# KKKSQJ/DeepLearning

Hardware: AMD Instinct MI355X
Metric: images/sec (higher is better)
Workload: dtype bf16; 1 GPU; model=resnet50, global_batch=256, image_size=224, parallelism=dp1

## Files before the change

csrc/batchnorm.hip:

```cpp
#include "common.h"
#include "vec.h"

namespace dla {


template <typename dev_t>
__global__ void bn_stats_kernel(const dev_t* __restrict__ x, float* __restrict__ sums,
                                int N, int C, int64_t HW) {
  __shared__ float smem[16];
  const int c = blockIdx.x;
  const int64_t total = (int64_t)N * HW;
  float sum = 0.f, sumsq = 0.f;
  for (int64_t m = (int64_t)blockIdx.y * blockDim.x + threadIdx.x; m < total;
       m += (int64_t)gridDim.y * blockDim.x) {
    const int64_t n = m / HW, hw = m % HW;
    const float f = to_f32(x[(n * C + c) * HW + hw]);
    sum += f;
    sumsq += f * f;
  }
  sum = block_reduce_sum(sum, smem);
  sumsq = block_reduce_sum(sumsq, smem);
  if (threadIdx.x == 0) {
    atomicAdd(&sums[c], sum);
    atomicAdd(&sums[C + c], sumsq);
  }
}

__device__ __forceinline__ void bn_finalize_channel(
    int c, float sum, float sumsq, const float* __restrict__ weight,
    const float* __restrict__ bias, float* __restrict__ mean,
    float* __restrict__ rstd, float* __restrict__ running_mean,
    float* __restrict__ running_var, float* __restrict__ scale,
    float* __restrict__ shift, float count, float eps, float momentum) {
  const float mu = sum / count;
  const float var = fmaxf(sumsq / count - mu * mu, 0.f);
  const float rs = rsqrtf(var + eps);
  mean[c] = mu;
  rstd[c] = rs;
  if (running_mean != nullptr && momentum > 0.f) {
    const float unbiased = var * count / fmaxf(count - 1.f, 1.f);
    running_mean[c] = (1.f - momentum) * running_mean[c] + momentum * mu;
    running_var[c] = (1.f - momentum) * running_var[c] + momentum * unbiased;
  }
  const float sc = weight[c] * rs;
  scale[c] = sc;
  shift[c] = bias[c] - mu * sc;
}

__global__ void bn_finalize_kernel(const float* __restrict__ sums,
                                   const float* __restrict__ weight,
                                   const float* __restrict__ bias,
                                   float* __restrict__ mean, float* __restrict__ rstd,
                                   float* __restrict__ running_mean,
                                   float* __restrict__ running_var,
                                   float* __restrict__ scale, float* __restrict__ shift,
                                   int C, float count, float eps, float momentum) {
  const int c = blockIdx.x * blockDim.x + threadIdx.x;
  if (c >= C) return;
  bn_finalize_channel(c, sums[c], sums[C + c], weight, bias, mean, rstd,
                      running_mean, running_var, scale, shift, count, eps,
                      momentum);
}

constexpr int kFinCh = 16, kFinRows = 64;

__global__ void __launch_bounds__(kFinCh * kFinRows)
bn_finalize_parts_kernel(const float* __restrict__ parts, int n_parts,
                         const float* __restrict__ weight,
                         const float* __restrict__ bias,
                         float* __restrict__ mean, float* __restrict__ rstd,
                         float* __restrict__ running_mean,
                         float* __restrict__ running_var,
                         float* __restrict__ scale, float* __restrict__ shift,
                         int C, float count, float eps, float momentum) {
  __shared__ float ls[2][kFinRows][kFinCh + 1];
  const int cl = threadIdx.x % kFinCh, rl = threadIdx.x / kFinCh;
  const int c = blockIdx.x * kFinCh + cl;
  float s = 0.f, q = 0.f;
  if (c < C) {
#pragma unroll 4
    for (int r = rl; r < n_parts; r += kFinRows) {
      const float* p = parts + (int64_t)r * 2 * C;
      s += p[c];
      q += p[C + c];
    }
  }
  ls[0][rl][cl] = s;
  ls[1][rl][cl] = q;
  __syncthreads();
  for (int h = kFinRows / 2; h > 0; h >>= 1) {
    if (rl < h) {
      ls[0][rl][cl] += ls[0][rl + h][cl];
      ls[1][rl][cl] += ls[1][rl + h][cl];
    }
    __syncthreads();
  }
  if (rl == 0 && c < C)
    bn_finalize_channel(c, ls[0][0][cl], ls[1][0][cl], weight, bias, mean,
                        rstd, running_mean, running_var, scale, shift, count,
                        eps, momentum);
}

template <typename dev_t, int V, bool RELU>
__global__ void bn_apply_kernel(const dev_t* __restrict__ x,
                                const float* __restrict__ scale,
                                const float* __restrict__ shift,
                                dev_t* __restrict__ y, int C, int64_t HW,
                                int64_t n_total) {
  const int64_t stride = (int64_t)gridDim.x * blockDim.x * V;
  for (int64_t i = ((int64_t)blockIdx.x * blockDim.x + threadIdx.x) * V;
       i < n_total; i += stride) {
    const int c = (int)((i / HW) % C);
    const float sc = scale[c], sh = shift[c];
    Vec<dev_t, V> xv = vload<dev_t, V>(x + i);
    Vec<dev_t, V> yv;
#pragma unroll
    for (int j = 0; j < V; ++j) {
      const float f = bn_pre(to_f32(xv.v[j]), sc, sh);
      yv.v[j] = from_f32<dev_t>(RELU ? fmaxf(f, 0.f) : f);
    }
    vstore<dev_t, V>(y + i, yv);
  }
}

template <typename dev_t, bool RELU>
__global__ void bn_bwd_stats_kernel(const dev_t* __restrict__ dy,
                                    const dev_t* __restrict__ x,
                                    const dev_t* __restrict__ y,
                                    const float* __restrict__ mean,
                                    const float* __restrict__ rstd,
                                    float* __restrict__ sums,
                                    int N, int C, int64_t HW) {
  __shared__ float smem[16];
  const int c = blockIdx.x;
  const float mu = mean[c], rs = rstd[c];
  const int64_t total = (int64_t)N * HW;
  float s_dy = 0.f, s_dyxh = 0.f;
  for (int64_t m = (int64_t)blockIdx.y * blockDim.x + threadIdx.x; m < total;
       m += (int64_t)gridDim.y * blockDim.x) {
    const int64_t n = m / HW, hw = m % HW;
    const int64_t idx = (n * C + c) * HW + hw;
    float g = to_f32(dy[idx]);
    if (RELU && to_f32(y[idx]) <= 0.f) g = 0.f;
    const float xh = (to_f32(x[idx]) - mu) * rs;
    s_dy += g;
    s_dyxh += g * xh;
  }
  s_dy = block_reduce_sum(s_dy, smem);
  s_dyxh = block_reduce_sum(s_dyxh, smem);
  if (threadIdx.x == 0) {
    atomicAdd(&sums[c], s_dy);
    atomicAdd(&sums[C + c], s_dyxh);
  }
}

template <typename dev_t, bool RELU>
__global__ void bn_bwd_dx_kernel(const dev_t* __restrict__ dy,
                                 const dev_t* __restrict__ x,
                                 const dev_t* __restrict__ y,
                                 const float* __restrict__ mean,
                                 const float* __restrict__ rstd,
                                 const float* __restrict__ weight,
                                 const float* __restrict__ sums,
                                 dev_t* __restrict__ dx, int C, int64_t HW,
                                 int64_t n_total, float inv_count) {
  const int64_t stride = (int64_t)gridDim.x * blockDim.x;
  for (int64_t i = (int64_t)blockIdx.x * blockDim.x + threadIdx.x; i < n_total;
       i += stride) {
    const int c = (int)((i / HW) % C);
    const float mu = mean[c], rs = rstd[c];
    float g = to_f32(dy[i]);
    if (RELU && to_f32(y[i]) <= 0.f) g = 0.f;
    const float xh = (to_f32(x[i]) - mu) * rs;
    const float m_dy = sums[c] * inv_count;
    const float m_dyxh = sums[C + c] * inv_count;
    dx[i] = from_f32<dev_t>(weight[c] * rs * (g - m_dy - xh * m_dyxh));
  }
}



inline int64_t nhwc_used_threads(int lanes_per_row, int64_t rows,
                                 int64_t target_lanes) {
  int64_t k = target_lanes / lanes_per_row;
  if (k > rows) k = rows;
  if (k < 1) k = 1;
  return (int64_t)lanes_per_row * k;
}

constexpr int kRedThreads = 256;
constexpr int kRedLanes = 32;
constexpr int kRedBlocks = 2048;
constexpr int kRedMaxParts = 512;
constexpr int kRedMinRows = 8;
constexpr int red_unroll(int tensors) { return tensors <= 2 ? 4 : 2; }

#define DLA_RED_KERNEL \
  __launch_bounds__(dla::kRedThreads) __attribute__((amdgpu_waves_per_eu(1, 4)))

struct NhwcRedTile {
  int bl, rb, chunks, parts;
};

inline NhwcRedTile nhwc_red_tile(int lanes_per_row, int64_t rows,
                                 int blocks = kRedBlocks,
                                 int max_parts = kRedMaxParts) {
  NhwcRedTile t;
  t.chunks = (lanes_per_row + kRedLanes - 1) / kRedLanes;
  t.bl = (lanes_per_row + t.chunks - 1) / t.chunks;
  t.rb = kRedThreads / t.bl;
  const int64_t per_part = (int64_t)t.rb * kRedMinRows;
  const int64_t by_rows = (rows + per_part - 1) / per_part;
  const int64_t p = std::min<int64_t>(
      std::min<int64_t>(blocks / t.chunks, max_parts), by_rows);
  t.parts = (int)std::max<int64_t>(p, 1);
  return t;
}

struct NhwcRedPos {
  int c0;
  int64_t row;
  int64_t rstride;
  bool active;
};

template <int V>
__device__ __forceinline__ NhwcRedPos nhwc_red_pos(int C, int bl, int rb) {
  const int lane = threadIdx.x % bl, rl = threadIdx.x / bl;
  const int gl = blockIdx.x * bl + lane;
  NhwcRedPos p;
  p.c0 = gl * V;
  p.row = (int64_t)blockIdx.y * rb + rl;
  p.rstride = (int64_t)gridDim.y * rb;
  p.active = rl < rb && gl < C / V;
  return p;
}

template <int U, typename L, typename A>
__device__ __forceinline__ void nhwc_red_rows(const NhwcRedPos& p,
                                              int64_t rows, L&& load, A&& add) {
  if (!p.active) return;
  using D = decltype(load(int64_t{}));
  int64_t r = p.row;
  for (; r + (U - 1) * p.rstride < rows; r += U * p.rstride) {
    D d[U];
#pragma unroll
    for (int u = 0; u < U; ++u) d[u] = load(r + u * p.rstride);
#pragma unroll
    for (int u = 0; u < U; ++u) add(r + u * p.rstride, d[u]);
  }
  for (; r < rows; r += p.rstride) add(r, load(r));
}

template <int V, int NS>
__device__ __forceinline__ void nhwc_red_tail(const float (&acc)[NS][V],
                                              float* __restrict__ slab, int C,
                                              int bl, int rb) {
  __shared__ __attribute__((aligned(16))) float ls[kRedThreads * V];
  const int W = bl * V;
  const int cbase = blockIdx.x * W;
  float* out = slab + (int64_t)blockIdx.y * NS * C;
#pragma unroll
  for (int s = 0; s < NS; ++s) {
    if (s) __syncthreads();
    if ((int)threadIdx.x < bl * rb) {
#pragma unroll
      for (int j = 0; j < V; ++j) ls[threadIdx.x * V + j] = acc[s][j];
    }
    __syncthreads();
    for (int col = threadIdx.x; col < W; col += kRedThreads) {
      if (cbase + col < C) {
        float sum = 0.f;
        for (int r = 0; r < rb; ++r) sum += ls[r * W + col];
        out[s * C + cbase + col] = sum;
      }
    }
  }
}

constexpr int kSlabCols = 32, kSlabRows = 32;

__global__ void __launch_bounds__(kSlabCols * kSlabRows)
bn_slab_reduce_kernel(const float* __restrict__ slab, int n_parts, int n_cols,
                      float* __restrict__ sums) {
  __shared__ float ls[kSlabRows][kSlabCols + 1];
  const int cl = threadIdx.x % kSlabCols, rl = threadIdx.x / kSlabCols;
  const int c = blockIdx.x * kSlabCols + cl;
  float s = 0.f;
  if (c < n_cols) {
#pragma unroll 4
    for (int r = rl; r < n_parts; r += kSlabRows)
      s += slab[(int64_t)r * n_cols + c];
  }
  ls[rl][cl] = s;
  __syncthreads();
  for (int h = kSlabRows / 2; h > 0; h >>= 1) {
    if (rl < h) ls[rl][cl] += ls[rl + h][cl];
    __syncthreads();
  }
  if (rl == 0 && c < n_cols) sums[c] = ls[0][cl];
}

constexpr int kSlabGroup = 128;
constexpr int kSlabDeep = kRedMaxParts;

__global__ void __launch_bounds__(kSlabCols * kSlabRows)
bn_slab_group_reduce_kernel(const float* __restrict__ slab, int n_parts,
                            int n_cols, float* __restrict__ groups) {
  __shared__ float ls[kSlabRows][kSlabCols + 1];
  const int cl = threadIdx.x % kSlabCols, rl = threadIdx.x / kSlabCols;
  const int c = blockIdx.x * kSlabCols + cl;
  const int r0 = blockIdx.y * kSlabGroup;
  const int r1 = r0 + kSlabGroup < n_parts ? r0 + kSlabGroup : n_parts;
  float s = 0.f;
  if (c < n_cols) {
#pragma unroll 4
    for (int r = r0 + rl; r < r1; r += kSlabRows)
      s += slab[(int64_t)r * n_cols + c];
  }
  ls[rl][cl] = s;
  __syncthreads();
  for (int h = kSlabRows / 2; h > 0; h >>= 1) {
    if (rl < h) ls[rl][cl] += ls[rl + h][cl];
    __syncthreads();
  }
  if (rl == 0 && c < n_cols) groups[(int64_t)blockIdx.y * n_cols + c] = ls[0][cl];
}

template <typename dev_t, int V>
__global__ void DLA_RED_KERNEL
bn_stats_nhwc_kernel(const dev_t* __restrict__ x, float* __restrict__ slab,
                     int C, int64_t rows, int bl, int rb) {
  const NhwcRedPos p = nhwc_red_pos<V>(C, bl, rb);
  float acc[2][V];
#pragma unroll
  for (int j = 0; j < V; ++j) { acc[0][j] = 0.f; acc[1][j] = 0.f; }
  nhwc_red_rows<red_unroll(1)>(
      p, rows, [&](int64_t r) { return vload<dev_t, V>(x + r * C + p.c0); },
      [&](int64_t, const Vec<dev_t, V>& xv) {
#pragma unroll
        for (int j = 0; j < V; ++j) {
          const float f = to_f32(xv.v[j]);
          acc[0][j] += f;
          acc[1][j] += f * f;
        }
      });
  nhwc_red_tail<V, 2>(acc, slab, C, bl, rb);
}

template <typename dev_t, int V, bool RELU>
__global__ void bn_apply_nhwc_kernel(const dev_t* __restrict__ x,
                                     const float* __restrict__ scale,
                                     const float* __restrict__ shift,
                                     dev_t* __restrict__ y, int C, int64_t rows,
                                     int64_t used) {
  const int64_t t = (int64_t)blockIdx.x * blockDim.x + threadIdx.x;
  if (t >= used) return;
  const int lanes_per_row = C / V;
  const int c0 = (int)(t % lanes_per_row) * V;
  const int64_t rstride = used / lanes_per_row;
  float sc[V], sh[V];
#pragma unroll
  for (int j = 0; j < V; ++j) { sc[j] = scale[c0 + j]; sh[j] = shift[c0 + j]; }
  for (int64_t r = t / lanes_per_row; r < rows; r += rstride) {
    Vec<dev_t, V> xv = vload<dev_t, V>(x + r * C + c0);
    Vec<dev_t, V> yv;
#pragma unroll
    for (int j = 0; j < V; ++j) {
      const float f = bn_pre(to_f32(xv.v[j]), sc[j], sh[j]);
      yv.v[j] = from_f32<dev_t>(RELU ? fmaxf(f, 0.f) : f);
    }
    vstore<dev_t, V>(y + r * C + c0, yv);
  }
}

template <typename dev_t, int V, bool RELU, bool MASK_Y = false>
__global__ void DLA_RED_KERNEL
bn_bwd_stats_nhwc_kernel(const dev_t* __restrict__ dy,
                         const dev_t* __restrict__ x,
                         const dev_t* __restrict__ y,
                         const float* __restrict__ scale,
                         const float* __restrict__ shift,
                         const float* __restrict__ mean,
                         const float* __restrict__ rstd,
                         float* __restrict__ slab, int C, int64_t rows, int bl,
                         int rb) {
  const NhwcRedPos p = nhwc_red_pos<V>(C, bl, rb);
  float mu[V], rs[V], sc[V], sh[V];
  float acc[2][V];
#pragma unroll
  for (int j = 0; j < V; ++j) {
    mu[j] = p.active ? mean[p.c0 + j] : 0.f;
    rs[j] = p.active ? rstd[p.c0 + j] : 0.f;
    sc[j] = (p.active && RELU && !MASK_Y) ? scale[p.c0 + j] : 0.f;
    sh[j] = (p.active && RELU && !MASK_Y) ? shift[p.c0 + j] : 0.f;
    acc[0][j] = 0.f;
    acc[1][j] = 0.f;
  }
  struct Row {
    Vec<dev_t, V> dy, x, y;
  };
  nhwc_red_rows<red_unroll(MASK_Y ? 3 : 2)>(
      p, rows,
      [&](int64_t r) {
        const int64_t base = r * C + p.c0;
        Row d;
        d.dy = vload<dev_t, V>(dy + base);
        d.x = vload<dev_t, V>(x + base);
        if (RELU && MASK_Y) d.y = vload<dev_t, V>(y + base);
        return d;
      },
      [&](int64_t, const Row& d) {
#pragma unroll
        for (int j = 0; j < V; ++j) {
          float g = to_f32(d.dy.v[j]);
          const float xf = to_f32(d.x.v[j]);
          if (RELU && MASK_Y && to_f32(d.y.v[j]) <= 0.f) g = 0.f;
          if (RELU && !MASK_Y && !(bn_pre(xf, sc[j], sh[j]) > 0.f)) g = 0.f;
          const float xh = (xf - mu[j]) * rs[j];
          acc[0][j] += g;
          acc[1][j] += g * xh;
        }
      });
  nhwc_red_tail<V, 2>(acc, slab, C, bl, rb);
}

template <typename dev_t, int V, bool RELU, bool MASK_Y = false>
__global__ void bn_bwd_dx_nhwc_kernel(const dev_t* __restrict__ dy,
                                      const dev_t* __restrict__ x,
                                      const dev_t* __restrict__ y,
                                      const float* __restrict__ scale,
                                      const float* __restrict__ shift,
                                      const float* __restrict__ mean,
                                      const float* __restrict__ rstd,
                                      const float* __restrict__ weight,
                                      const float* __restrict__ sums,
                                      dev_t* __restrict__ dx, int C,
                                      int64_t rows, int64_t used,
                                      float inv_count) {
  const int64_t t = (int64_t)blockIdx.x * blockDim.x + threadIdx.x;
  if (t >= used) return;
  const int lanes_per_row = C / V;
  const int c0 = (int)(t % lanes_per_row) * V;
  const int64_t rstride = used / lanes_per_row;
  float mu[V], rs[V], wr[V], sc[V], sh[V], m_dy[V], m_dyxh[V];
#pragma unroll
  for (int j = 0; j < V; ++j) {
    mu[j] = mean[c0 + j];
    rs[j] = rstd[c0 + j];
    wr[j] = weight[c0 + j] * rs[j];
    sc[j] = (RELU && !MASK_Y) ? scale[c0 + j] : 0.f;
    sh[j] = (RELU && !MASK_Y) ? shift[c0 + j] : 0.f;
    m_dy[j] = sums[c0 + j] * inv_count;
    m_dyxh[j] = sums[C + c0 + j] * inv_count;
  }
  for (int64_t r = t / lanes_per_row; r < rows; r += rstride) {
    const int64_t base = r * C + c0;
    Vec<dev_t, V> dyv = vload<dev_t, V>(dy + base);
    Vec<dev_t, V> xv = vload<dev_t, V>(x + base);
    Vec<dev_t, V> yv;
    if (RELU && MASK_Y) yv = vload<dev_t, V>(y + base);
    Vec<dev_t, V> dxv;
#pragma unroll
    for (int j = 0; j < V; ++j) {
      float g = to_f32(dyv.v[j]);
      const float xf = to_f32(xv.v[j]);
      if (RELU && MASK_Y && to_f32(yv.v[j]) <= 0.f) g = 0.f;
      if (RELU && !MASK_Y && !(bn_pre(xf, sc[j], sh[j]) > 0.f)) g = 0.f;
      const float xh = (xf - mu[j]) * rs[j];
      dxv.v[j] = from_f32<dev_t>(wr[j] * (g - m_dy[j] - xh * m_dyxh[j]));
    }
    vstore<dev_t, V>(dx + r * C + c0, dxv);
  }
}

template <typename dev_t, int V, bool DUAL>
__global__ void bn_add_relu_nhwc_kernel(const dev_t* __restrict__ x,
                                        const float* __restrict__ scale,
                                        const float* __restrict__ shift,
                                        const dev_t* __restrict__ idn,
                                        const float* __restrict__ scale_d,
                                        const float* __restrict__ shift_d,
                                        dev_t* __restrict__ out, int C,
                                        int64_t rows, int64_t used) {
  const int64_t t = (int64_t)blockIdx.x * blockDim.x + threadIdx.x;
  if (t >= used) return;
  const int lanes_per_row = C / V;
  const int c0 = (int)(t % lanes_per_row) * V;
  const int64_t rstride = used / lanes_per_row;
  float sc[V], sh[V], scd[V];
#pragma unroll
  for (int j = 0; j < V; ++j) {
    sc[j] = scale[c0 + j];
    sh[j] = shift[c0 + j];
    if (DUAL) {
      scd[j] = scale_d[c0 + j];
      sh[j] += shift_d[c0 + j];
    }
  }
  for (int64_t r = t / lanes_per_row; r < rows; r += rstride) {
    const int64_t base = r * C + c0;
    Vec<dev_t, V> xv = vload<dev_t, V>(x + base);
    Vec<dev_t, V> iv = vload<dev_t, V>(idn + base);
    Vec<dev_t, V> ov;
#pragma unroll
    for (int j = 0; j < V; ++j) {
      float f = to_f32(xv.v[j]) * sc[j] + sh[j];
      f += DUAL ? to_f32(iv.v[j]) * scd[j] : to_f32(iv.v[j]);
      ov.v[j] = from_f32<dev_t>(fmaxf(f, 0.f));
    }
    vstore<dev_t, V>(out + base, ov);
  }
}

template <typename dev_t, int V, bool DUAL>
__global__ void DLA_RED_KERNEL
bn_join_bwd_stats_nhwc_kernel(
    const dev_t* __restrict__ dy, const dev_t* __restrict__ out,
    const dev_t* __restrict__ x, const float* __restrict__ mean,
    const float* __restrict__ rstd, const dev_t* __restrict__ xd,
    const float* __restrict__ mean_d, const float* __restrict__ rstd_d,
    dev_t* __restrict__ g_out, float* __restrict__ slab, int C, int64_t rows,
    int bl, int rb) {
  constexpr int NS = DUAL ? 3 : 2;
  const NhwcRedPos p = nhwc_red_pos<V>(C, bl, rb);
  float mu[V], rs[V], mud[V], rsd[V];
  float acc[NS][V];
#pragma unroll
  for (int j = 0; j < V; ++j) {
    mu[j] = p.active ? mean[p.c0 + j] : 0.f;
    rs[j] = p.active ? rstd[p.c0 + j] : 0.f;
    mud[j] = (p.active && DUAL) ? mean_d[p.c0 + j] : 0.f;
    rsd[j] = (p.active && DUAL) ? rstd_d[p.c0 + j] : 0.f;
#pragma unroll
    for (int s = 0; s < NS; ++s) acc[s][j] = 0.f;
  }
  struct Row {
    Vec<dev_t, V> dy, out, x, xd;
  };
  nhwc_red_rows<red_unroll(DUAL ? 4 : 3)>(
      p, rows,
      [&](int64_t r) {
        const int64_t base = r * C + p.c0;
        Row d;
        d.dy = vload<dev_t, V>(dy + base);
        d.out = vload<dev_t, V>(out + base);
        d.x = vload<dev_t, V>(x + base);
        if (DUAL) d.xd = vload<dev_t, V>(xd + base);
        return d;
      },
      [&](int64_t r, const Row& d) {
        Vec<dev_t, V> gv;
#pragma unroll
        for (int j = 0; j < V; ++j) {
          const bool on = to_f32(d.out.v[j]) > 0.f;
          gv.v[j] = on ? d.dy.v[j] : from_f32<dev_t>(0.f);
          const float g = on ? to_f32(d.dy.v[j]) : 0.f;
          acc[0][j] += g;
          acc[1][j] += g * ((to_f32(d.x.v[j]) - mu[j]) * rs[j]);
          if (DUAL)
            acc[NS - 1][j] += g * ((to_f32(d.xd.v[j]) - mud[j]) * rsd[j]);
        }
        vstore<dev_t, V>(g_out + r * C + p.c0, gv);
      });
  nhwc_red_tail<V, NS>(acc, slab, C, bl, rb);
}

template <typename dev_t, int V>
__global__ void bn_join_bwd_dx_dual_nhwc_kernel(
    const dev_t* __restrict__ g, const dev_t* __restrict__ x,
    const dev_t* __restrict__ xd, const float* __restrict__ mean,
    const float* __restrict__ rstd, const float* __restrict__ weight,
    const float* __restrict__ mean_d, const float* __restrict__ rstd_d,
    const float* __restrict__ weight_d, const float* __restrict__ sums,
    dev_t* __restrict__ dx, dev_t* __restrict__ dxd, int C, int64_t rows,
    int64_t used, float inv_count) {
  const int64_t t = (int64_t)blockIdx.x * blockDim.x + threadIdx.x;
  if (t >= used) return;
  const int lanes_per_row = C / V;
  const int c0 = (int)(t % lanes_per_row) * V;
  const int64_t rstride = used / lanes_per_row;
  float mu[V], rs[V], wr[V], mud[V], rsd[V], wrd[V], m_g[V], m_gxh[V],
      m_gxhd[V];
#pragma unroll
  for (int j = 0; j < V; ++j) {
    mu[j] = mean[c0 + j];
    rs[j] = rstd[c0 + j];
    wr[j] = weight[c0 + j] * rs[j];
    mud[j] = mean_d[c0 + j];
    rsd[j] = rstd_d[c0 + j];
    wrd[j] = weight_d[c0 + j] * rsd[j];
    m_g[j] = sums[c0 + j] * inv_count;
    m_gxh[j] = sums[C + c0 + j] * inv_count;
    m_gxhd[j] = sums[2 * C + c0 + j] * inv_count;
  }
  for (int64_t r = t / lanes_per_row; r < rows; r += rstride) {
    const int64_t base = r * C + c0;
    Vec<dev_t, V> gv = vload<dev_t, V>(g + base);
    Vec<dev_t, V> xv = vload<dev_t, V>(x + base);
    Vec<dev_t, V> xdv = vload<dev_t, V>(xd + base);
    Vec<dev_t, V> dxv, dxdv;
#pragma unroll
    for (int j = 0; j < V; ++j) {
      const float gg = to_f32(gv.v[j]) - m_g[j];
      const float xh = (to_f32(xv.v[j]) - mu[j]) * rs[j];
      const float xhd = (to_f32(xdv.v[j]) - mud[j]) * rsd[j];
      dxv.v[j] = from_f32<dev_t>(wr[j] * (gg - xh * m_gxh[j]));
      dxdv.v[j] = from_f32<dev_t>(wrd[j] * (gg - xhd * m_gxhd[j]));
    }
    vstore<dev_t, V>(dx + base, dxv);
    vstore<dev_t, V>(dxd + base, dxdv);
  }
}

inline bool is_nhwc(const torch::Tensor& t) {
  return t.dim() == 4 && t.is_contiguous(at::MemoryFormat::ChannelsLast) &&
         !t.is_contiguous();
}

struct BnFinalized {
  torch::Tensor mean, rstd, scale, shift;
};

inline BnFinalized bn_finalize_launch(
    const torch::Tensor& sums, const torch::Tensor& weight,
    const torch::Tensor& bias, c10::optional<torch::Tensor>& running_mean,
    c10::optional<torch::Tensor>& running_var, int C, int64_t rows,
    double momentum, double eps) {
  TORCH_CHECK(sums.is_cuda() && sums.scalar_type() == torch::kFloat &&
                  sums.is_contiguous(),
              "bn sums must be a contiguous fp32 GPU tensor");
  TORCH_CHECK((sums.dim() == 1 && sums.size(0) == 2 * C) ||
                  (sums.dim() == 2 && sums.size(0) >= 1 &&
                   sums.size(1) == 2 * C),
              "bn sums must be [2C] or [n_parts, 2C]");
  TORCH_CHECK(weight.numel() == C && bias.numel() == C,
              "bn weight/bias must have C elements");
  auto opts_f = sums.options();
  BnFinalized f{torch::empty({C}, opts_f), torch::empty({C}, opts_f),
                torch::empty({C}, opts_f), torch::empty({C}, opts_f)};
  auto w32 = weight.to(torch::kFloat).contiguous();
  auto b32 = bias.to(torch::kFloat).contiguous();
  float* rm = running_mean.has_value() ? running_mean->data_ptr<float>() : nullptr;
  float* rv = running_var.has_value() ? running_var->data_ptr<float>() : nullptr;
  const int n_parts = sums.dim() == 2 ? (int)sums.size(0) : 1;
  if (n_parts > 1) {
    hipLaunchKernelGGL(bn_finalize_parts_kernel, dim3((C + kFinCh - 1) / kFinCh),
                       dim3(kFinCh * kFinRows), 0, stream(),
                       sums.data_ptr<float>(), n_parts, w32.data_ptr<float>(),
                       b32.data_ptr<float>(), f.mean.data_ptr<float>(),
                       f.rstd.data_ptr<float>(), rm, rv,
                       f.scale.data_ptr<float>(), f.shift.data_ptr<float>(), C,
                       (float)rows, (float)eps, (float)momentum);
  } else {
    hipLaunchKernelGGL(bn_finalize_kernel, dim3((C + 255) / 256), dim3(256), 0,
                       stream(), sums.data_ptr<float>(), w32.data_ptr<float>(),
                       b32.data_ptr<float>(), f.mean.data_ptr<float>(),
                       f.rstd.data_ptr<float>(), rm, rv,
                       f.scale.data_ptr<float>(), f.shift.data_ptr<float>(), C,
                       (float)rows, (float)eps, (float)momentum);
  }
  return f;
}

inline torch::Tensor bn_param_grad(const torch::Tensor& sums, int64_t offset,
                                   int C, const torch::Tensor& weight) {
  return sums.narrow(0, offset, C).to(weight.scalar_type());
}

inline torch::Tensor bn_slab_reduce_launch(const torch::Tensor& slab) {
  const int n_parts = (int)slab.size(0), n_cols = (int)slab.size(1);
  if (n_parts > kSlabDeep) {
    const int groups = (n_parts + kSlabGroup - 1) / kSlabGroup;
    auto part = torch::empty({groups, n_cols}, slab.options());
    hipLaunchKernelGGL(bn_slab_group_reduce_kernel,
                       dim3((n_cols + kSlabCols - 1) / kSlabCols, groups),
                       dim3(kSlabCols * kSlabRows), 0, stream(),
                       slab.data_ptr<float>(), n_parts, n_cols,
                       part.data_ptr<float>());
    return bn_slab_reduce_launch(part);
  }
  auto sums = torch::empty({n_cols}, slab.options());
  hipLaunchKernelGGL(bn_slab_reduce_kernel,
                     dim3((n_cols + kSlabCols - 1) / kSlabCols),
                     dim3(kSlabCols * kSlabRows), 0, stream(),
                     slab.data_ptr<float>(), n_parts, n_cols,
                     sums.data_ptr<float>());
  return sums;
}

inline bool is_nhwc_rows(const torch::Tensor& t) {
  return t.dim() == 4 && t.is_contiguous(at::MemoryFormat::ChannelsLast);
}

}

std::vector<torch::Tensor> batchnorm_fwd(torch::Tensor x, torch::Tensor weight,
                                         torch::Tensor bias,
                                         c10::optional<torch::Tensor> running_mean,
                                         c10::optional<torch::Tensor> running_var,
                                         double momentum, double eps, bool relu) {
  DLA_CHECK_CUDA(x);
  TORCH_CHECK(x.dim() == 4, "batchnorm_fwd expects a 4D tensor");
  const bool nhwc = dla::is_nhwc(x);
  TORCH_CHECK(nhwc || x.is_contiguous(), "batchnorm_fwd: x must be contiguous "
              "(NCHW or channels_last)");
  const int N = (int)x.size(0), C = (int)x.size(1);
  const int64_t HW = x.size(2) * x.size(3);
  auto opts_f = x.options().dtype(torch::kFloat);
  auto sums = nhwc ? torch::Tensor() : torch::zeros({2 * C}, opts_f);
  auto mean = torch::empty({C}, opts_f);
  auto rstd = torch::empty({C}, opts_f);
  auto scale = torch::empty({C}, opts_f);
  auto shift = torch::empty({C}, opts_f);
  auto y = torch::empty_like(x);
  auto w32 = weight.to(torch::kFloat);
  auto b32 = bias.to(torch::kFloat);

  const int64_t rows = (int64_t)N * HW;
  const int ysplit = (int)std::min<int64_t>((rows + 65535) / 65536 + 1,
                                            std::max(1, 2048 / C));
  DLA_DISPATCH_FLOAT_TYPES(x.scalar_type(), "batchnorm_fwd", [&] {
    if (nhwc) {
      constexpr int VM = 16 / (int)sizeof(dev_t);
      auto stats = [&](auto vtag) {
        constexpr int V = decltype(vtag)::value;
        const auto t = dla::nhwc_red_tile(C / V, rows);
        sums = torch::empty({t.parts, 2 * C}, opts_f);
        hipLaunchKernelGGL((dla::bn_stats_nhwc_kernel<dev_t, V>),
                           dim3(t.chunks, t.parts), dim3(dla::kRedThreads), 0,
                           dla::stream(), (const dev_t*)x.data_ptr(),
                           sums.data_ptr<float>(), C, rows, t.bl, t.rb);
      };
      if (C % VM == 0) stats(std::integral_constant<int, VM>{});
      else if (C % 2 == 0) stats(std::integral_constant<int, 2>{});
      else stats(std::integral_constant<int, 1>{});
    } else {
      hipLaunchKernelGGL((dla::bn_stats_kernel<dev_t>), dim3(C, ysplit), dim3(256), 0,
                         dla::stream(), (const dev_t*)x.data_ptr(),
                         sums.data_ptr<float>(), N, C, HW);
    }
    float* rm = running_mean.has_value() ? running_mean->data_ptr<float>() : nullptr;
    float* rv = running_var.has_value() ? running_var->data_ptr<float>() : nullptr;
    if (sums.dim() == 2 && sums.size(0) > 1) {
      hipLaunchKernelGGL(dla::bn_finalize_parts_kernel,
                         dim3((C + dla::kFinCh - 1) / dla::kFinCh),
                         dim3(dla::kFinCh * dla::kFinRows), 0, dla::stream(),
                         sums.data_ptr<float>(), (int)sums.size(0),
                         w32.data_ptr<float>(), b32.data_ptr<float>(),
                         mean.data_ptr<float>(), rstd.data_ptr<float>(), rm, rv,
                         scale.data_ptr<float>(), shift.data_ptr<float>(), C,
                         (float)rows, (float)eps, (float)momentum);
    } else {
      hipLaunchKernelGGL(dla::bn_finalize_kernel, dim3((C + 255) / 256), dim3(256), 0,
                         dla::stream(), sums.data_ptr<float>(), w32.data_ptr<float>(),
                         b32.data_ptr<float>(), mean.data_ptr<float>(),
                         rstd.data_ptr<float>(), rm, rv,
                         scale.data_ptr<float>(), shift.data_ptr<float>(), C,
                         (float)rows, (float)eps, (float)momentum);
    }
    const int64_t n_total = x.numel();
    constexpr int VMAX = 16 / (int)sizeof(dev_t);
    auto launch = [&](auto vtag, auto rtag) {
      constexpr int V = decltype(vtag)::value;
      constexpr bool R = decltype(rtag)::value;
      if (nhwc) {
        const int lanes = C / V;
        const int64_t used = dla::nhwc_used_threads(lanes, rows, 524288);
        hipLaunchKernelGGL((dla::bn_apply_nhwc_kernel<dev_t, V, R>),
                           dim3((int)((used + 255) / 256)), dim3(256), 0,
                           dla::stream(), (const dev_t*)x.data_ptr(),
                           scale.data_ptr<float>(), shift.data_ptr<float>(),
                           (dev_t*)y.data_ptr(), C, rows, used);
        return;
      }
      const int grid = dla::grid_1d((n_total + V - 1) / V, 256);
      if (false) ;
      else
        hipLaunchKernelGGL((dla::bn_apply_kernel<dev_t, V, R>), dim3(grid), dim3(256),
                           0, dla::stream(), (const dev_t*)x.data_ptr(),
                           scale.data_ptr<float>(), shift.data_ptr<float>(),
                           (dev_t*)y.data_ptr(), C, HW, n_total);
    };
    const bool vec_ok = nhwc ? (C % VMAX == 0) : (HW % VMAX == 0);
    if (vec_ok) {
      if (relu) launch(std::integral_constant<int, VMAX>{}, std::true_type{});
      else launch(std::integral_constant<int, VMAX>{}, std::false_type{});
    } else {
      if (relu) launch(std::integral_constant<int, 1>{}, std::true_type{});
      else launch(std::integral_constant<int, 1>{}, std::false_type{});
    }
  });
  HIP_CHECK_ERR();
  return {y, mean, rstd, scale, shift};
}

std::vector<torch::Tensor> batchnorm_fwd_from_sums(
    torch::Tensor x, torch::Tensor weight, torch::Tensor bias,
    torch::Tensor sums, c10::optional<torch::Tensor> running_mean,
    c10::optional<torch::Tensor> running_var, double momentum, double eps,
    bool relu) {
  DLA_CHECK_CUDA(x);
  TORCH_CHECK(x.dim() == 4, "batchnorm_fwd_from_sums expects a 4D tensor");
  const bool nhwc = dla::is_nhwc(x);
  TORCH_CHECK(nhwc || x.is_contiguous(),
              "batchnorm_fwd_from_sums: x must be contiguous");
  const int N = (int)x.size(0), C = (int)x.size(1);
  const int64_t HW = x.size(2) * x.size(3);
  auto y = torch::empty_like(x);
  const int64_t rows = (int64_t)N * HW;
  auto fin = dla::bn_finalize_launch(sums, weight, bias, running_mean,
                                     running_var, C, rows, momentum, eps);
  auto& mean = fin.mean;
  auto& rstd = fin.rstd;
  auto& scale = fin.scale;
  auto& shift = fin.shift;
  DLA_DISPATCH_FLOAT_TYPES(x.scalar_type(), "batchnorm_fwd_from_sums", [&] {
    const int64_t n_total = x.numel();
    constexpr int VMAX = 16 / (int)sizeof(dev_t);
    auto launch = [&](auto vtag, auto rtag) {
      constexpr int V = decltype(vtag)::value;
      constexpr bool R = decltype(rtag)::value;
      if (nhwc) {
        const int lanes = C / V;
        const int64_t used = dla::nhwc_used_threads(lanes, rows, 524288);
        hipLaunchKernelGGL((dla::bn_apply_nhwc_kernel<dev_t, V, R>),
                           dim3((int)((used + 255) / 256)), dim3(256), 0,
                           dla::stream(), (const dev_t*)x.data_ptr(),
                           scale.data_ptr<float>(), shift.data_ptr<float>(),
                           (dev_t*)y.data_ptr(), C, rows, used);
        return;
      }
      const int grid = dla::grid_1d((n_total + V - 1) / V, 256);
      hipLaunchKernelGGL((dla::bn_apply_kernel<dev_t, V, R>), dim3(grid),
                         dim3(256), 0, dla::stream(),
                         (const dev_t*)x.data_ptr(), scale.data_ptr<float>(),
                         shift.data_ptr<float>(), (dev_t*)y.data_ptr(), C, HW,
                         n_total);
    };
    const bool vec_ok = nhwc ? (C % VMAX == 0) : (HW % VMAX == 0);
    if (vec_ok) {
      if (relu) launch(std::integral_constant<int, VMAX>{}, std::true_type{});
      else launch(std::integral_constant<int, VMAX>{}, std::false_type{});
    } else {
      if (relu) launch(std::integral_constant<int, 1>{}, std::true_type{});
      else launch(std::integral_constant<int, 1>{}, std::false_type{});
    }
  });
  HIP_CHECK_ERR();
  return {y, mean, rstd, scale, shift};
}

torch::Tensor bn_apply(torch::Tensor x, torch::Tensor scale, torch::Tensor shift,
                       bool relu) {
  DLA_CHECK_CUDA(x);
  TORCH_CHECK(x.dim() == 4, "bn_apply expects a 4D tensor");
  const bool nhwc = dla::is_nhwc(x);
  TORCH_CHECK(nhwc || x.is_contiguous(), "bn_apply: x must be contiguous");
  const int C = (int)x.size(1);
  const int64_t HW = x.size(2) * x.size(3);
  auto y = torch::empty_like(x);
  auto sc = scale.to(torch::kFloat).contiguous();
  auto sh = shift.to(torch::kFloat).contiguous();
  const int64_t n_total = x.numel();
  DLA_DISPATCH_FLOAT_TYPES(x.scalar_type(), "bn_apply", [&] {
    constexpr int VMAX = 16 / (int)sizeof(dev_t);
    auto launch = [&](auto vtag, auto rtag) {
      constexpr int V = decltype(vtag)::value;
      constexpr bool R = decltype(rtag)::value;
      if (nhwc) {
        const int64_t rows = n_total / C;
        const int lanes = C / V;
        const int64_t used = dla::nhwc_used_threads(lanes, rows, 524288);
        hipLaunchKernelGGL((dla::bn_apply_nhwc_kernel<dev_t, V, R>),
                           dim3((int)((used + 255) / 256)), dim3(256), 0,
                           dla::stream(), (const dev_t*)x.data_ptr(),
                           sc.data_ptr<float>(), sh.data_ptr<float>(),
                           (dev_t*)y.data_ptr(), C, rows, used);
        return;
      }
      const int grid = dla::grid_1d((n_total + V - 1) / V, 256);
      if (false) ;
      else
        hipLaunchKernelGGL((dla::bn_apply_kernel<dev_t, V, R>), dim3(grid), dim3(256),
                           0, dla::stream(), (const dev_t*)x.data_ptr(),
                           sc.data_ptr<float>(), sh.data_ptr<float>(),
                           (dev_t*)y.data_ptr(), C, HW, n_total);
    };
    const bool vec_ok = nhwc ? (C % VMAX == 0) : (HW % VMAX == 0);
    if (vec_ok) {
      if (relu) launch(std::integral_constant<int, VMAX>{}, std::true_type{});
      else launch(std::integral_constant<int, VMAX>{}, std::false_type{});
    } else {
      if (relu) launch(std::integral_constant<int, 1>{}, std::true_type{});
      else launch(std::integral_constant<int, 1>{}, std::false_type{});
    }
  });
  HIP_CHECK_ERR();
  return y;
}

bool bn_relu_mask_from_x(torch::Tensor x) { return dla::is_nhwc(x); }

std::vector<torch::Tensor> batchnorm_bwd_ex(
    torch::Tensor dy, torch::Tensor x, c10::optional<torch::Tensor> y,
    torch::Tensor weight, torch::Tensor mean, torch::Tensor rstd,
    c10::optional<torch::Tensor> scale, c10::optional<torch::Tensor> shift,
    bool relu) {
  DLA_CHECK_CUDA(dy); DLA_CHECK_CUDA(x);
  const bool nhwc = dla::is_nhwc(x);
  TORCH_CHECK(nhwc || x.is_contiguous(), "batchnorm_bwd: x must be contiguous");
  if (nhwc && !dla::is_nhwc(dy)) dy = dy.contiguous(at::MemoryFormat::ChannelsLast);
  if (!nhwc) dy = dy.contiguous();
  const int N = (int)x.size(0), C = (int)x.size(1);
  const int64_t HW = x.size(2) * x.size(3);
  const int64_t rows = (int64_t)N * HW;
  auto opts_f = x.options().dtype(torch::kFloat);
  auto sums = nhwc ? torch::Tensor() : torch::zeros({2 * C}, opts_f);
  auto dx = torch::empty_like(x);
  auto w32 = weight.to(torch::kFloat);
  const int ysplit = (int)std::min<int64_t>((rows + 65535) / 65536 + 1,
                                            std::max(1, 2048 / C));
  const bool mask_y = relu && y.has_value();
  if (relu && !mask_y) {
    TORCH_CHECK(bn_relu_mask_from_x(x) && scale.has_value() && shift.has_value(),
                "batchnorm_bwd: the relu mask needs y, or channels_last x "
                "with the forward's scale and shift");
    for (const auto* t : {&*scale, &*shift})
      TORCH_CHECK(t->is_cuda() && t->scalar_type() == torch::kFloat &&
                      t->is_contiguous() && t->numel() == C,
                  "batchnorm_bwd: scale/shift must be contiguous fp32 [C]");
  }
  if (mask_y)
    TORCH_CHECK(y->scalar_type() == x.scalar_type() && y->sizes() == x.sizes() &&
                    (nhwc ? dla::is_nhwc(*y) : y->is_contiguous()),
                "batchnorm_bwd: y must match x (shape, dtype, layout)");
  const float* scp = (relu && !mask_y) ? scale->data_ptr<float>() : nullptr;
  const float* shp = (relu && !mask_y) ? shift->data_ptr<float>() : nullptr;
  DLA_DISPATCH_FLOAT_TYPES(x.scalar_type(), "batchnorm_bwd", [&] {
    const dev_t* yp = mask_y ? (const dev_t*)y->data_ptr() : nullptr;
    auto with_mode = [&](auto f) {
      if (!relu) f(std::false_type{}, std::false_type{});
      else if (mask_y) f(std::true_type{}, std::true_type{});
      else f(std::true_type{}, std::false_type{});
    };
    with_mode([&](auto rtag, auto mtag) {
      constexpr bool R = decltype(rtag)::value;
      constexpr bool MY = decltype(mtag)::value;
      if (nhwc) {
        constexpr int VM = 16 / (int)sizeof(dev_t);
        auto stats = [&](auto vtag) {
          constexpr int V = decltype(vtag)::value;
          const auto t = dla::nhwc_red_tile(C / V, rows);
          auto slab = torch::empty({t.parts, 2 * C}, opts_f);
          hipLaunchKernelGGL((dla::bn_bwd_stats_nhwc_kernel<dev_t, V, R, MY>),
                             dim3(t.chunks, t.parts), dim3(dla::kRedThreads),
                             0, dla::stream(), (const dev_t*)dy.data_ptr(),
                             (const dev_t*)x.data_ptr(), yp, scp, shp,
                             mean.data_ptr<float>(), rstd.data_ptr<float>(),
                             slab.data_ptr<float>(), C, rows, t.bl, t.rb);
          sums = dla::bn_slab_reduce_launch(slab);
        };
        if (C % VM == 0) stats(std::integral_constant<int, VM>{});
        else if (C % 2 == 0) stats(std::integral_constant<int, 2>{});
        else stats(std::integral_constant<int, 1>{});
      } else if constexpr (!R || MY) {
        hipLaunchKernelGGL((dla::bn_bwd_stats_kernel<dev_t, R>), dim3(C, ysplit),
                           dim3(256), 0, dla::stream(), (const dev_t*)dy.data_ptr(),
                           (const dev_t*)x.data_ptr(), yp, mean.data_ptr<float>(),
                           rstd.data_ptr<float>(), sums.data_ptr<float>(), N, C, HW);
      }
    });

    const int64_t n_total = x.numel();
    const float inv_count = 1.f / (float)rows;
    constexpr int VMAX = 16 / (int)sizeof(dev_t);
    with_mode([&](auto rtag, auto mtag) {
      constexpr bool R = decltype(rtag)::value;
      constexpr bool MY = decltype(mtag)::value;
      if (nhwc) {
        auto dxk = [&](auto vtag) {
          constexpr int V = decltype(vtag)::value;
          const int lanes = C / V;
          const int64_t used = dla::nhwc_used_threads(lanes, rows, 524288);
          hipLaunchKernelGGL((dla::bn_bwd_dx_nhwc_kernel<dev_t, V, R, MY>),
                             dim3((int)((used + 255) / 256)), dim3(256), 0,
                             dla::stream(), (const dev_t*)dy.data_ptr(),
                             (const dev_t*)x.data_ptr(), yp, scp, shp,
                             mean.data_ptr<float>(), rstd.data_ptr<float>(),
                             w32.data_ptr<float>(), sums.data_ptr<float>(),
                             (dev_t*)dx.data_ptr(), C, rows, used, inv_count);
        };
        if (C % VMAX == 0) dxk(std::integral_constant<int, VMAX>{});
        else dxk(std::integral_constant<int, 1>{});
      } else if constexpr (!R || MY) {
        hipLaunchKernelGGL((dla::bn_bwd_dx_kernel<dev_t, R>), dim3(dla::grid_1d(n_total, 256)),
                           dim3(256), 0, dla::stream(), (const dev_t*)dy.data_ptr(),
                           (const dev_t*)x.data_ptr(), yp, mean.data_ptr<float>(),
                           rstd.data_ptr<float>(), w32.data_ptr<float>(),
                           sums.data_ptr<float>(), (dev_t*)dx.data_ptr(), C, HW,
                           n_total, inv_count);
      }
    });
  });
  HIP_CHECK_ERR();
  return {dx, dla::bn_param_grad(sums, C, C, weight),
          dla::bn_param_grad(sums, 0, C, weight)};
}

std::vector<torch::Tensor> batchnorm_bwd(torch::Tensor dy, torch::Tensor x,
                                         c10::optional<torch::Tensor> y,
                                         torch::Tensor weight, torch::Tensor mean,
                                         torch::Tensor rstd, bool relu) {
  TORCH_CHECK(!relu || y.has_value(), "batchnorm_bwd: relu mask needs y");
  return batchnorm_bwd_ex(dy, x, relu ? y : c10::nullopt, weight, mean, rstd,
                          c10::nullopt, c10::nullopt, relu);
}

namespace dla {

inline void join_check(const torch::Tensor& x, const torch::Tensor& other,
                       const char* what) {
  TORCH_CHECK(other.is_cuda() && other.scalar_type() == x.scalar_type() &&
                  other.sizes() == x.sizes() && is_nhwc_rows(other),
              "bn join: ", what, " must match x (shape, dtype, channels_last)");
}

inline int join_vec(const torch::Tensor& x) {
  const int vmax = 16 / (int)x.element_size();
  TORCH_CHECK(x.size(1) % vmax == 0,
              "bn join: C must be a multiple of ", vmax);
  return vmax;
}

}

std::vector<torch::Tensor> bn_add_relu_fwd_from_sums(
    torch::Tensor x, torch::Tensor weight, torch::Tensor bias,
    torch::Tensor sums, c10::optional<torch::Tensor> running_mean,
    c10::optional<torch::Tensor> running_var, double momentum, double eps,
    torch::Tensor identity) {
  DLA_CHECK_CUDA(x);
  TORCH_CHECK(dla::is_nhwc_rows(x), "bn_add_relu: x must be channels_last");
  dla::join_check(x, identity, "identity");
  dla::join_vec(x);
  const int C = (int)x.size(1);
  const int64_t rows = x.numel() / C;
  auto fin = dla::bn_finalize_launch(sums, weight, bias, running_mean,
                                     running_var, C, rows, momentum, eps);
  auto out = torch::empty_like(x);
  DLA_DISPATCH_FLOAT_TYPES(x.scalar_type(), "bn_add_relu_fwd_from_sums", [&] {
    constexpr int V = 16 / (int)sizeof(dev_t);
    const int64_t used = dla::nhwc_used_threads(C / V, rows, 524288);
    hipLaunchKernelGGL((dla::bn_add_relu_nhwc_kernel<dev_t, V, false>),
                       dim3((int)((used + 255) / 256)), dim3(256), 0,
                       dla::stream(), (const dev_t*)x.data_ptr(),
                       fin.scale.data_ptr<float>(), fin.shift.data_ptr<float>(),
                       (const dev_t*)identity.data_ptr(), nullptr, nullptr,
                       (dev_t*)out.data_ptr(), C, rows, used);
  });
  HIP_CHECK_ERR();
  return {out, fin.mean, fin.rstd};
}

std::vector<torch::Tensor> bn_add_relu_dual_fwd_from_sums(
    torch::Tensor x, torch::Tensor weight, torch::Tensor bias,
    torch::Tensor sums, c10::optional<torch::Tensor> running_mean,
    c10::optional<torch::Tensor> running_var, double momentum, double eps,
    torch::Tensor xd, torch::Tensor weight_d, torch::Tensor bias_d,
    torch::Tensor sums_d, c10::optional<torch::Tensor> running_mean_d,
    c10::optional<torch::Tensor> running_var_d, double momentum_d,
    double eps_d) {
  DLA_CHECK_CUDA(x);
  TORCH_CHECK(dla::is_nhwc_rows(x), "bn_add_relu_dual: x must be channels_last");
  dla::join_check(x, xd, "xd");
  dla::join_vec(x);
  const int C = (int)x.size(1);
  const int64_t rows = x.numel() / C;
  auto fin = dla::bn_finalize_launch(sums, weight, bias, running_mean,
                                     running_var, C, rows, momentum, eps);
  auto fd = dla::bn_finalize_launch(sums_d, weight_d, bias_d, running_mean_d,
                                    running_var_d, C, rows, momentum_d, eps_d);
  auto out = torch::empty_like(x);
  DLA_DISPATCH_FLOAT_TYPES(x.scalar_type(), "bn_add_relu_dual_fwd_from_sums", [&] {
    constexpr int V = 16 / (int)sizeof(dev_t);
    const int64_t used = dla::nhwc_used_threads(C / V, rows, 524288);
    hipLaunchKernelGGL((dla::bn_add_relu_nhwc_kernel<dev_t, V, true>),
                       dim3((int)((used + 255) / 256)), dim3(256), 0,
                       dla::stream(), (const dev_t*)x.data_ptr(),
                       fin.scale.data_ptr<float>(), fin.shift.data_ptr<float>(),
                       (const dev_t*)xd.data_ptr(), fd.scale.data_ptr<float>(),
                       fd.shift.data_ptr<float>(), (dev_t*)out.data_ptr(), C,
                       rows, used);
  });
  HIP_CHECK_ERR();
  return {out, fin.mean, fin.rstd, fd.mean, fd.rstd};
}

std::vector<torch::Tensor> bn_add_relu_bwd(torch::Tensor dy, torch::Tensor out,
                                           torch::Tensor x, torch::Tensor weight,
                                           torch::Tensor mean,
                                           torch::Tensor rstd) {
  DLA_CHECK_CUDA(x);
  TORCH_CHECK(dla::is_nhwc_rows(x), "bn_add_relu_bwd: x must be channels_last");
  dla::join_check(x, out, "out");
  if (!dla::is_nhwc_rows(dy)) dy = dy.contiguous(at::MemoryFormat::ChannelsLast);
  dla::join_check(x, dy, "dy");
  dla::join_vec(x);
  const int C = (int)x.size(1);
  const int64_t rows = x.numel() / C;
  TORCH_CHECK(mean.numel() == C && rstd.numel() == C && weight.numel() == C,
              "bn_add_relu_bwd: per-channel tensors must have C elements");
  torch::Tensor sums;
  auto g = torch::empty_like(x);
  auto dx = torch::empty_like(x);
  auto w32 = weight.to(torch::kFloat).contiguous();
  DLA_DISPATCH_FLOAT_TYPES(x.scalar_type(), "bn_add_relu_bwd", [&] {
    constexpr int V = 16 / (int)sizeof(dev_t);
    const int lanes = C / V;
    const auto t = dla::nhwc_red_tile(lanes, rows);
    auto slab = torch::empty({t.parts, 2 * C},
                             x.options().dtype(torch::kFloat));
    hipLaunchKernelGGL((dla::bn_join_bwd_stats_nhwc_kernel<dev_t, V, false>),
                       dim3(t.chunks, t.parts), dim3(dla::kRedThreads), 0,
                       dla::stream(),
                       (const dev_t*)dy.data_ptr(), (const dev_t*)out.data_ptr(),
                       (const dev_t*)x.data_ptr(), mean.data_ptr<float>(),
                       rstd.data_ptr<float>(), nullptr, nullptr, nullptr,
                       (dev_t*)g.data_ptr(), slab.data_ptr<float>(), C, rows,
                       t.bl, t.rb);
    sums = dla::bn_slab_reduce_launch(slab);
    const int64_t used = dla::nhwc_used_threads(lanes, rows, 524288);
    hipLaunchKernelGGL((dla::bn_bwd_dx_nhwc_kernel<dev_t, V, false>),
                       dim3((int)((used + 255) / 256)), dim3(256), 0,
                       dla::stream(), (const dev_t*)g.data_ptr(),
                       (const dev_t*)x.data_ptr(), nullptr, nullptr, nullptr,
                       mean.data_ptr<float>(), rstd.data_ptr<float>(),
                       w32.data_ptr<float>(), sums.data_ptr<float>(),
                       (dev_t*)dx.data_ptr(), C, rows, used,
                       1.f / (float)rows);
  });
  HIP_CHECK_ERR();
  return {g, dx, dla::bn_param_grad(sums, C, C, weight),
          dla::bn_param_grad(sums, 0, C, weight)};
}

std::vector<torch::Tensor> bn_add_relu_dual_bwd(
    torch::Tensor dy, torch::Tensor out, torch::Tensor x, torch::Tensor weight,
    torch::Tensor mean, torch::Tensor rstd, torch::Tensor xd,
    torch::Tensor weight_d, torch::Tensor mean_d, torch::Tensor rstd_d) {
  DLA_CHECK_CUDA(x);
  TORCH_CHECK(dla::is_nhwc_rows(x), "bn_add_relu_dual_bwd: x must be channels_last");
  dla::join_check(x, out, "out");
  dla::join_check(x, xd, "xd");
  if (!dla::is_nhwc_rows(dy)) dy = dy.contiguous(at::MemoryFormat::ChannelsLast);
  dla::join_check(x, dy, "dy");
  dla::join_vec(x);
  const int C = (int)x.size(1);
  const int64_t rows = x.numel() / C;
  TORCH_CHECK(mean.numel() == C && rstd.numel() == C && weight.numel() == C &&
                  mean_d.numel() == C && rstd_d.numel() == C &&
                  weight_d.numel() == C,
              "bn_add_relu_dual_bwd: per-channel tensors must have C elements");
  torch::Tensor sums;
  auto g = torch::empty_like(x);
  auto dx = torch::empty_like(x);
  auto dxd = torch::empty_like(x);
  auto w32 = weight.to(torch::kFloat).contiguous();
  auto wd32 = weight_d.to(torch::kFloat).contiguous();
  DLA_DISPATCH_FLOAT_TYPES(x.scalar_type(), "bn_add_relu_dual_bwd", [&] {
    constexpr int V = 16 / (int)sizeof(dev_t);
    const int lanes = C / V;
    const auto t = dla::nhwc_red_tile(lanes, rows);
    auto slab = torch::empty({t.parts, 3 * C},
                             x.options().dtype(torch::kFloat));
    hipLaunchKernelGGL((dla::bn_join_bwd_stats_nhwc_kernel<dev_t, V, true>),
                       dim3(t.chunks, t.parts), dim3(dla::kRedThreads), 0,
                       dla::stream(),
                       (const dev_t*)dy.data_ptr(), (const dev_t*)out.data_ptr(),
                       (const dev_t*)x.data_ptr(), mean.data_ptr<float>(),
                       rstd.data_ptr<float>(), (const dev_t*)xd.data_ptr(),
                       mean_d.data_ptr<float>(), rstd_d.data_ptr<float>(),
                       (dev_t*)g.data_ptr(), slab.data_ptr<float>(), C, rows,
                       t.bl, t.rb);
    sums = dla::bn_slab_reduce_launch(slab);
    const int64_t used = dla::nhwc_used_threads(lanes, rows, 524288);
    hipLaunchKernelGGL((dla::bn_join_bwd_dx_dual_nhwc_kernel<dev_t, V>),
                       dim3((int)((used + 255) / 256)), dim3(256), 0,
                       dla::stream(), (const dev_t*)g.data_ptr(),
                       (const dev_t*)x.data_ptr(), (const dev_t*)xd.data_ptr(),
                       mean.data_ptr<float>(), rstd.data_ptr<float>(),
                       w32.data_ptr<float>(), mean_d.data_ptr<float>(),
                       rstd_d.data_ptr<float>(), wd32.data_ptr<float>(),
                       sums.data_ptr<float>(), (dev_t*)dx.data_ptr(),
                       (dev_t*)dxd.data_ptr(), C, rows, used,
                       1.f / (float)rows);
  });
  HIP_CHECK_ERR();
  auto dbias = dla::bn_param_grad(sums, 0, C, weight);
  return {dx, dxd, dla::bn_param_grad(sums, C, C, weight), dbias,
          dla::bn_param_grad(sums, 2 * C, C, weight_d),
          dbias.to(weight_d.scalar_type()).clone()};
}

namespace dla {

inline void dx_only_check(const torch::Tensor& x, const torch::Tensor& g,
                          const torch::Tensor& slab, int ns) {
  TORCH_CHECK(is_nhwc_rows(x), "bn dx-only: x must be channels_last");
  join_check(x, g, "g");
  TORCH_CHECK(x.scalar_type() == torch::kBFloat16, "bn dx-only: bf16 only");
  TORCH_CHECK(slab.is_cuda() && slab.scalar_type() == torch::kFloat &&
                  slab.dim() == 2 && slab.is_contiguous() &&
                  slab.size(0) >= 1 && slab.size(1) == ns * x.size(1),
              "bn dx-only: slab must be fp32 [n_parts, ", ns, "*C]");
}

}

torch::Tensor bn_slab_reduce(torch::Tensor slab) {
  TORCH_CHECK(slab.is_cuda() && slab.scalar_type() == torch::kFloat &&
                  slab.dim() == 2 && slab.is_contiguous() && slab.size(0) >= 1,
              "bn_slab_reduce: slab must be a contiguous fp32 [n_parts, n_cols] "
              "GPU tensor");
  auto sums = dla::bn_slab_reduce_launch(slab);
  HIP_CHECK_ERR();
  return sums;
}

std::vector<torch::Tensor> bn_bwd_dx_from_slab(torch::Tensor g,
                                               torch::Tensor slab,
                                               torch::Tensor x,
                                               torch::Tensor weight,
                                               torch::Tensor mean,
                                               torch::Tensor rstd) {
  DLA_CHECK_CUDA(x);
  dla::dx_only_check(x, g, slab, 2);
  const int V = dla::join_vec(x);
  const int C = (int)x.size(1);
  const int64_t rows = x.numel() / C;
  TORCH_CHECK(mean.numel() == C && rstd.numel() == C && weight.numel() == C,
              "bn_bwd_dx_from_slab: per-channel tensors must have C elements");
  auto dx = torch::empty_like(x);
  auto w32 = weight.to(torch::kFloat).contiguous();
  auto sums = dla::bn_slab_reduce_launch(slab);
  using dev_t = __hip_bfloat16;
  const int64_t used = dla::nhwc_used_threads(C / V, rows, 524288);
  hipLaunchKernelGGL((dla::bn_bwd_dx_nhwc_kernel<dev_t, 8, false>),
                     dim3((int)((used + 255) / 256)), dim3(256), 0,
                     dla::stream(), (const dev_t*)g.data_ptr(),
                     (const dev_t*)x.data_ptr(), nullptr, nullptr, nullptr,
                     mean.data_ptr<float>(), rstd.data_ptr<float>(),
                     w32.data_ptr<float>(), sums.data_ptr<float>(),
                     (dev_t*)dx.data_ptr(), C, rows, used, 1.f / (float)rows);
  HIP_CHECK_ERR();
  return {dx, dla::bn_param_grad(sums, C, C, weight),
          dla::bn_param_grad(sums, 0, C, weight)};
}

std::vector<torch::Tensor> bn_join_dual_bwd_dx_from_slab(
    torch::Tensor g, torch::Tensor slab, torch::Tensor x, torch::Tensor weight,
    torch::Tensor mean, torch::Tensor rstd, torch::Tensor xd,
    torch::Tensor weight_d, torch::Tensor mean_d, torch::Tensor rstd_d) {
  DLA_CHECK_CUDA(x);
  dla::dx_only_check(x, g, slab, 3);
  dla::join_check(x, xd, "xd");
  const int V = dla::join_vec(x);
  const int C = (int)x.size(1);
  const int64_t rows = x.numel() / C;
  TORCH_CHECK(mean.numel() == C && rstd.numel() == C && weight.numel() == C &&
                  mean_d.numel() == C && rstd_d.numel() == C &&
                  weight_d.numel() == C,
              "bn_join_dual_bwd_dx_from_slab: per-channel tensors must have C "
              "elements");
  auto dx = torch::empty_like(x);
  auto dxd = torch::empty_like(x);
  auto w32 = weight.to(torch::kFloat).contiguous();
  auto wd32 = weight_d.to(torch::kFloat).contiguous();
  auto sums = dla::bn_slab_reduce_launch(slab);
  using dev_t = __hip_bfloat16;
  const int64_t used = dla::nhwc_used_threads(C / V, rows, 524288);
  hipLaunchKernelGGL((dla::bn_join_bwd_dx_dual_nhwc_kernel<dev_t, 8>),
                     dim3((int)((used + 255) / 256)), dim3(256), 0,
                     dla::stream(), (const dev_t*)g.data_ptr(),
                     (const dev_t*)x.data_ptr(), (const dev_t*)xd.data_ptr(),
                     mean.data_ptr<float>(), rstd.data_ptr<float>(),
                     w32.data_ptr<float>(), mean_d.data_ptr<float>(),
                     rstd_d.data_ptr<float>(), wd32.data_ptr<float>(),
                     sums.data_ptr<float>(), (dev_t*)dx.data_ptr(),
                     (dev_t*)dxd.data_ptr(), C, rows, used,
                     1.f / (float)rows);
  HIP_CHECK_ERR();
  auto dbias = dla::bn_param_grad(sums, 0, C, weight);
  return {dx, dxd, dla::bn_param_grad(sums, C, C, weight), dbias,
          dla::bn_param_grad(sums, 2 * C, C, weight_d),
          dbias.to(weight_d.scalar_type()).clone()};
}

namespace dla {

constexpr int kPoolRun = 8;

template <typename dev_t, int V>
__global__ void __launch_bounds__(256)
bn_relu_maxpool_fwd_nhwc_kernel(const dev_t* __restrict__ x,
                                const float* __restrict__ scale,
                                const float* __restrict__ shift,
                                dev_t* __restrict__ out,
                                uint8_t* __restrict__ slots, int C, int H,
                                int W, int OH, int OW, int runs_per_img) {
  const int n = blockIdx.x / runs_per_img;
  const int oh0 = (blockIdx.x % runs_per_img) * kPoolRun;
  const int oh1 = min(oh0 + kPoolRun, OH);
  const int lanes = C / V;
  const int items = (oh1 - oh0) * OW * lanes;
  const dev_t* xn = x + (int64_t)n * H * W * C;
  const int64_t obase = ((int64_t)n * OH + oh0) * OW * C;
  for (int i = threadIdx.x; i < items; i += blockDim.x) {
    const int c0 = (i % lanes) * V;
    const int p = i / lanes;
    const int ow = p % OW, oh = oh0 + p / OW;
    float sc[V], sh[V], best[V];
    int slot[V];
#pragma unroll
    for (int j = 0; j < V; ++j) {
      sc[j] = scale[c0 + j];
      sh[j] = shift[c0 + j];
      best[j] = -INFINITY;
      slot[j] = 4;
    }
#pragma unroll
    for (int kh = 0; kh < 3; ++kh) {
      const int ih = 2 * oh - 1 + kh;
      if (ih < 0 || ih >= H) continue;
#pragma unroll
      for (int kw = 0; kw < 3; ++kw) {
        const int iw = 2 * ow - 1 + kw;
        if (iw < 0 || iw >= W) continue;
        Vec<dev_t, V> xv =
            vload<dev_t, V>(xn + ((int64_t)ih * W + iw) * C + c0);
#pragma unroll
        for (int j = 0; j < V; ++j) {
          const float f = bn_pre(to_f32(xv.v[j]), sc[j], sh[j]);
          const float y = to_f32(from_f32<dev_t>(fmaxf(f, 0.f)));
          if (y > best[j]) {
            best[j] = y;
            slot[j] = kh * 3 + kw;
          }
        }
      }
    }
    Vec<dev_t, V> ov;
    Vec<uint8_t, V> sv;
#pragma unroll
    for (int j = 0; j < V; ++j) {
      ov.v[j] = from_f32<dev_t>(best[j]);
      sv.v[j] = (uint8_t)slot[j];
    }
    const int64_t o = obase + (int64_t)p * C + c0;
    vstore<dev_t, V>(out + o, ov);
    vstore<uint8_t, V>(slots + o, sv);
  }
}

template <typename dev_t, int V>
__device__ __forceinline__ void stem_pool_grad(
    const dev_t* __restrict__ dpool, const uint8_t* __restrict__ slots,
    const Vec<dev_t, V>& xv, const float* sc, const float* sh, int n, int h,
    int w, int c0, int C, int OH, int OW, float* g) {
#pragma unroll
  for (int j = 0; j < V; ++j) g[j] = 0.f;
  const int oh_hi = min((h + 1) >> 1, OH - 1);
  const int ow_hi = min((w + 1) >> 1, OW - 1);
  for (int oh = h >> 1; oh <= oh_hi; ++oh) {
    const int kh = h - 2 * oh + 1;
    for (int ow = w >> 1; ow <= ow_hi; ++ow) {
      const int want = kh * 3 + (w - 2 * ow + 1);
      const int64_t o = (((int64_t)n * OH + oh) * OW + ow) * C + c0;
      Vec<uint8_t, V> sv = vload<uint8_t, V>(slots + o);
      Vec<dev_t, V> dv = vload<dev_t, V>(dpool + o);
#pragma unroll
      for (int j = 0; j < V; ++j)
        if ((int)sv.v[j] == want) g[j] += to_f32(dv.v[j]);
    }
  }
#pragma unroll
  for (int j = 0; j < V; ++j)
    if (!(bn_pre(to_f32(xv.v[j]), sc[j], sh[j]) > 0.f)) g[j] = 0.f;
}

constexpr int kStemRedBlocks = 1024;

template <typename dev_t, int V>
__global__ void __launch_bounds__(kRedThreads)
bn_relu_maxpool_bwd_stats_nhwc_kernel(
    const dev_t* __restrict__ dpool, const uint8_t* __restrict__ slots,
    const dev_t* __restrict__ x, const float* __restrict__ scale,
    const float* __restrict__ shift, const float* __restrict__ mean,
    const float* __restrict__ rstd, float* __restrict__ slab, int C, int H,
    int W, int OH, int OW, int64_t rows, int bl, int rb) {
  const NhwcRedPos p = nhwc_red_pos<V>(C, bl, rb);
  float mu[V], rs[V], sc[V], sh[V];
  float acc[2][V];
#pragma unroll
  for (int j = 0; j < V; ++j) {
    mu[j] = p.active ? mean[p.c0 + j] : 0.f;
    rs[j] = p.active ? rstd[p.c0 + j] : 0.f;
    sc[j] = p.active ? scale[p.c0 + j] : 0.f;
    sh[j] = p.active ? shift[p.c0 + j] : 0.f;
    acc[0][j] = 0.f;
    acc[1][j] = 0.f;
  }
  nhwc_red_rows<1>(
      p, rows, [&](int64_t r) { return vload<dev_t, V>(x + r * C + p.c0); },
      [&](int64_t r, const Vec<dev_t, V>& xv) {
        const uint32_t r32 = (uint32_t)r;
        const uint32_t q = r32 / (uint32_t)W;
        const int w = (int)(r32 - q * (uint32_t)W);
        const int n = (int)(q / (uint32_t)H);
        const int h = (int)(q - (uint32_t)n * (uint32_t)H);
        float g[V];
        stem_pool_grad<dev_t, V>(dpool, slots, xv, sc, sh, n, h, w, p.c0, C,
                                 OH, OW, g);
#pragma unroll
        for (int j = 0; j < V; ++j) {
          const float xh = (to_f32(xv.v[j]) - mu[j]) * rs[j];
          acc[0][j] += g[j];
          acc[1][j] += g[j] * xh;
        }
      });
  nhwc_red_tail<V, 2>(acc, slab, C, bl, rb);
}

template <typename dev_t, int V>
__global__ void bn_relu_maxpool_bwd_dx_nhwc_kernel(
    const dev_t* __restrict__ dpool, const uint8_t* __restrict__ slots,
    const dev_t* __restrict__ x, const float* __restrict__ scale,
    const float* __restrict__ shift, const float* __restrict__ mean,
    const float* __restrict__ rstd, const float* __restrict__ weight,
    const float* __restrict__ sums, dev_t* __restrict__ dx, int C, int H,
    int W, int OH, int OW, int64_t rows, int64_t used, float inv_count) {
  const int64_t t = (int64_t)blockIdx.x * blockDim.x + threadIdx.x;
  if (t >= used) return;
  const int lanes_per_row = C / V;
  const int c0 = (int)(t % lanes_per_row) * V;
  const int64_t rstride = used / lanes_per_row;
  float mu[V], rs[V], wr[V], sc[V], sh[V], m_g[V], m_gxh[V], g[V];
#pragma unroll
  for (int j = 0; j < V; ++j) {
    mu[j] = mean[c0 + j];
    rs[j] = rstd[c0 + j];
    wr[j] = weight[c0 + j] * rs[j];
    sc[j] = scale[c0 + j];
    sh[j] = shift[c0 + j];
    m_g[j] = sums[c0 + j] * inv_count;
    m_gxh[j] = sums[C + c0 + j] * inv_count;
  }
  for (int64_t r = t / lanes_per_row; r < rows; r += rstride) {
    const uint32_t r32 = (uint32_t)r;
    const uint32_t q = r32 / (uint32_t)W;
    const int w = (int)(r32 - q * (uint32_t)W);
    const int n = (int)(q / (uint32_t)H);
    const int h = (int)(q - (uint32_t)n * (uint32_t)H);
    Vec<dev_t, V> xv = vload<dev_t, V>(x + r * C + c0);
    stem_pool_grad<dev_t, V>(dpool, slots, xv, sc, sh, n, h, w, c0, C, OH, OW,
                             g);
    Vec<dev_t, V> dxv;
#pragma unroll
    for (int j = 0; j < V; ++j) {
      const float xh = (to_f32(xv.v[j]) - mu[j]) * rs[j];
      dxv.v[j] = from_f32<dev_t>(wr[j] * (g[j] - m_g[j] - xh * m_gxh[j]));
    }
    vstore<dev_t, V>(dx + r * C + c0, dxv);
  }
}

inline void stem_check(const torch::Tensor& x, const char* fn) {
  TORCH_CHECK(x.is_cuda() && x.dim() == 4 && is_nhwc_rows(x), fn,
              ": x must be a channels_last 4D GPU tensor");
  const int vmax = 16 / (int)x.element_size();
  TORCH_CHECK(x.size(1) % vmax == 0, fn, ": C must be a multiple of ", vmax);
  TORCH_CHECK(x.numel() > 0 && x.numel() / x.size(1) < (int64_t(1) << 31),
              fn, ": N*H*W must be in [1, 2^31)");
}

}

std::vector<torch::Tensor> bn_relu_maxpool_fwd(
    torch::Tensor x, torch::Tensor weight, torch::Tensor bias,
    c10::optional<torch::Tensor> running_mean,
    c10::optional<torch::Tensor> running_var, double momentum, double eps) {
  dla::stem_check(x, "bn_relu_maxpool_fwd");
  const int N = (int)x.size(0), C = (int)x.size(1);
  const int H = (int)x.size(2), W = (int)x.size(3);
  const int OH = (H - 1) / 2 + 1, OW = (W - 1) / 2 + 1;
  const int64_t rows = (int64_t)N * H * W;
  auto out_opts = x.options().memory_format(at::MemoryFormat::ChannelsLast);
  auto pooled = torch::empty({N, C, OH, OW}, out_opts);
  auto slots = torch::empty({N, C, OH, OW}, out_opts.dtype(torch::kByte));
  const int runs = (OH + dla::kPoolRun - 1) / dla::kPoolRun;
  TORCH_CHECK((int64_t)N * runs < (int64_t(1) << 31),
              "bn_relu_maxpool_fwd: too many blocks");
  dla::BnFinalized fin;
  DLA_DISPATCH_FLOAT_TYPES(x.scalar_type(), "bn_relu_maxpool_fwd", [&] {
    constexpr int V = 16 / (int)sizeof(dev_t);
    const auto t = dla::nhwc_red_tile(C / V, rows);
    auto sums = torch::empty({t.parts, 2 * C},
                             x.options().dtype(torch::kFloat));
    hipLaunchKernelGGL((dla::bn_stats_nhwc_kernel<dev_t, V>),
                       dim3(t.chunks, t.parts), dim3(dla::kRedThreads), 0,
                       dla::stream(), (const dev_t*)x.data_ptr(),
                       sums.data_ptr<float>(), C, rows, t.bl, t.rb);
    fin = dla::bn_finalize_launch(sums, weight, bias, running_mean,
                                  running_var, C, rows, momentum, eps);
    hipLaunchKernelGGL((dla::bn_relu_maxpool_fwd_nhwc_kernel<dev_t, V>),
                       dim3(N * runs), dim3(256), 0, dla::stream(),
                       (const dev_t*)x.data_ptr(), fin.scale.data_ptr<float>(),
                       fin.shift.data_ptr<float>(), (dev_t*)pooled.data_ptr(),
                       slots.data_ptr<uint8_t>(), C, H, W, OH, OW, runs);
  });
  HIP_CHECK_ERR();
  return {pooled, slots, fin.mean, fin.rstd, fin.scale, fin.shift};
}

std::vector<torch::Tensor> bn_relu_maxpool_bwd(
    torch::Tensor dpool, torch::Tensor x, torch::Tensor slots,
    torch::Tensor weight, torch::Tensor mean, torch::Tensor rstd,
    torch::Tensor scale, torch::Tensor shift) {
  dla::stem_check(x, "bn_relu_maxpool_bwd");
  const int N = (int)x.size(0), C = (int)x.size(1);
  const int H = (int)x.size(2), W = (int)x.size(3);
  const int OH = (H - 1) / 2 + 1, OW = (W - 1) / 2 + 1;
  const int64_t rows = (int64_t)N * H * W;
  DLA_CHECK_CUDA(dpool);
  if (!dla::is_nhwc_rows(dpool))
    dpool = dpool.contiguous(at::MemoryFormat::ChannelsLast);
  const std::vector<int64_t> pshape{N, C, OH, OW};
  TORCH_CHECK(dpool.scalar_type() == x.scalar_type() &&
                  dpool.sizes() == at::IntArrayRef(pshape),
              "bn_relu_maxpool_bwd: dpool must be [N, C, OH, OW] of x's dtype");
  TORCH_CHECK(slots.is_cuda() && slots.scalar_type() == torch::kByte &&
                  slots.sizes() == at::IntArrayRef(pshape) &&
                  dla::is_nhwc_rows(slots),
              "bn_relu_maxpool_bwd: slots must be channels_last uint8 "
              "[N, C, OH, OW]");
  for (const auto* t : {&mean, &rstd, &scale, &shift})
    TORCH_CHECK(t->is_cuda() && t->scalar_type() == torch::kFloat &&
                    t->is_contiguous() && t->numel() == C,
                "bn_relu_maxpool_bwd: per-channel tensors must be contiguous "
                "fp32 [C]");
  TORCH_CHECK(weight.numel() == C, "bn_relu_maxpool_bwd: weight must be [C]");
  torch::Tensor sums;
  auto dx = torch::empty_like(x);
  auto w32 = weight.to(torch::kFloat).contiguous();
  DLA_DISPATCH_FLOAT_TYPES(x.scalar_type(), "bn_relu_maxpool_bwd", [&] {
    constexpr int V = 16 / (int)sizeof(dev_t);
    const int lanes = C / V;
    const auto t = dla::nhwc_red_tile(lanes, rows, dla::kStemRedBlocks,
                                      dla::kStemRedBlocks);
    auto slab = torch::empty({t.parts, 2 * C},
                             x.options().dtype(torch::kFloat));
    hipLaunchKernelGGL((dla::bn_relu_maxpool_bwd_stats_nhwc_kernel<dev_t, V>),
                       dim3(t.chunks, t.parts), dim3(dla::kRedThreads), 0,
                       dla::stream(), (const dev_t*)dpool.data_ptr(),
                       slots.data_ptr<uint8_t>(), (const dev_t*)x.data_ptr(),
                       scale.data_ptr<float>(), shift.data_ptr<float>(),
                       mean.data_ptr<float>(), rstd.data_ptr<float>(),
                       slab.data_ptr<float>(), C, H, W, OH, OW, rows, t.bl,
                       t.rb);
    sums = dla::bn_slab_reduce_launch(slab);
    const int64_t used = dla::nhwc_used_threads(lanes, rows, 524288);
    hipLaunchKernelGGL((dla::bn_relu_maxpool_bwd_dx_nhwc_kernel<dev_t, V>),
                       dim3((int)((used + 255) / 256)), dim3(256), 0,
                       dla::stream(), (const dev_t*)dpool.data_ptr(),
                       slots.data_ptr<uint8_t>(), (const dev_t*)x.data_ptr(),
                       scale.data_ptr<float>(), shift.data_ptr<float>(),
                       mean.data_ptr<float>(), rstd.data_ptr<float>(),
                       w32.data_ptr<float>(), sums.data_ptr<float>(),
                       (dev_t*)dx.data_ptr(), C, H, W, OH, OW, rows, used,
                       1.f / (float)rows);
  });
  HIP_CHECK_ERR();
  return {dx, dla::bn_param_grad(sums, C, C, weight),
          dla::bn_param_grad(sums, 0, C, weight)};
}
```

csrc/bindings.cpp:

```cpp
#include <torch/extension.h>

std::vector<torch::Tensor> layernorm_fwd(torch::Tensor x, torch::Tensor w,
                                         torch::Tensor b, double eps);
std::vector<torch::Tensor> layernorm_bwd(torch::Tensor dy, torch::Tensor x,
                                         torch::Tensor w, torch::Tensor mean,
                                         torch::Tensor rstd);
torch::Tensor gelu_fwd(torch::Tensor x);
torch::Tensor gelu_bwd(torch::Tensor dy, torch::Tensor x);
torch::Tensor silu_fwd(torch::Tensor x);
torch::Tensor silu_bwd(torch::Tensor dy, torch::Tensor x);
torch::Tensor add_relu_fwd(torch::Tensor a, torch::Tensor b);
torch::Tensor relu_mask_bwd(torch::Tensor dy, torch::Tensor y);
std::vector<torch::Tensor> batchnorm_fwd(torch::Tensor x, torch::Tensor weight,
                                         torch::Tensor bias,
                                         c10::optional<torch::Tensor> running_mean,
                                         c10::optional<torch::Tensor> running_var,
                                         double momentum, double eps, bool relu);
torch::Tensor bn_apply(torch::Tensor x, torch::Tensor scale, torch::Tensor shift,
                       bool relu);
std::vector<torch::Tensor> batchnorm_bwd(torch::Tensor dy, torch::Tensor x,
                                         c10::optional<torch::Tensor> y,
                                         torch::Tensor weight, torch::Tensor mean,
                                         torch::Tensor rstd, bool relu);
bool bn_relu_mask_from_x(torch::Tensor x);
std::vector<torch::Tensor> batchnorm_bwd_ex(
    torch::Tensor dy, torch::Tensor x, c10::optional<torch::Tensor> y,
    torch::Tensor weight, torch::Tensor mean, torch::Tensor rstd,
    c10::optional<torch::Tensor> scale, c10::optional<torch::Tensor> shift,
    bool relu);
std::vector<torch::Tensor> bn_relu_maxpool_fwd(
    torch::Tensor x, torch::Tensor weight, torch::Tensor bias,
    c10::optional<torch::Tensor> running_mean,
    c10::optional<torch::Tensor> running_var, double momentum, double eps);
std::vector<torch::Tensor> bn_relu_maxpool_bwd(
    torch::Tensor dpool, torch::Tensor x, torch::Tensor slots,
    torch::Tensor weight, torch::Tensor mean, torch::Tensor rstd,
    torch::Tensor scale, torch::Tensor shift);
std::vector<torch::Tensor> batchnorm_fwd_from_sums(
    torch::Tensor x, torch::Tensor weight, torch::Tensor bias,
    torch::Tensor sums, c10::optional<torch::Tensor> running_mean,
    c10::optional<torch::Tensor> running_var, double momentum, double eps,
    bool relu);
std::vector<torch::Tensor> bn_add_relu_fwd_from_sums(
    torch::Tensor x, torch::Tensor weight, torch::Tensor bias,
    torch::Tensor sums, c10::optional<torch::Tensor> running_mean,
    c10::optional<torch::Tensor> running_var, double momentum, double eps,
    torch::Tensor identity);
std::vector<torch::Tensor> bn_add_relu_dual_fwd_from_sums(
    torch::Tensor x, torch::Tensor weight, torch::Tensor bias,
    torch::Tensor sums, c10::optional<torch::Tensor> running_mean,
    c10::optional<torch::Tensor> running_var, double momentum, double eps,
    torch::Tensor xd, torch::Tensor weight_d, torch::Tensor bias_d,
    torch::Tensor sums_d, c10::optional<torch::Tensor> running_mean_d,
    c10::optional<torch::Tensor> running_var_d, double momentum_d,
    double eps_d);
std::vector<torch::Tensor> bn_add_relu_bwd(torch::Tensor dy, torch::Tensor out,
                                           torch::Tensor x, torch::Tensor weight,
                                           torch::Tensor mean,
                                           torch::Tensor rstd);
std::vector<torch::Tensor> bn_add_relu_dual_bwd(
    torch::Tensor dy, torch::Tensor out, torch::Tensor x, torch::Tensor weight,
    torch::Tensor mean, torch::Tensor rstd, torch::Tensor xd,
    torch::Tensor weight_d, torch::Tensor mean_d, torch::Tensor rstd_d);
torch::Tensor bn_slab_reduce(torch::Tensor slab);
std::vector<torch::Tensor> bn_bwd_dx_from_slab(torch::Tensor g,
                                               torch::Tensor slab,
                                               torch::Tensor x,
                                               torch::Tensor weight,
                                               torch::Tensor mean,
                                               torch::Tensor rstd);
std::vector<torch::Tensor> bn_join_dual_bwd_dx_from_slab(
    torch::Tensor g, torch::Tensor slab, torch::Tensor x, torch::Tensor weight,
    torch::Tensor mean, torch::Tensor rstd, torch::Tensor xd,
    torch::Tensor weight_d, torch::Tensor mean_d, torch::Tensor rstd_d);
std::vector<torch::Tensor> conv1x1_dgrad_bwdstats(
    torch::Tensor dy, torch::Tensor wt, c10::optional<torch::Tensor> residual,
    int64_t mode, c10::optional<torch::Tensor> out, torch::Tensor x,
    c10::optional<torch::Tensor> scale, c10::optional<torch::Tensor> shift,
    torch::Tensor mean, torch::Tensor rstd, c10::optional<torch::Tensor> xd,
    c10::optional<torch::Tensor> mean_d, c10::optional<torch::Tensor> rstd_d);
std::vector<torch::Tensor> conv1x1_fwd(torch::Tensor a, torch::Tensor b,
                                       c10::optional<torch::Tensor> bias,
                                       c10::optional<torch::Tensor> scale,
                                       c10::optional<torch::Tensor> shift,
                                       c10::optional<torch::Tensor> residual,
                                       bool relu, bool want_stats);
torch::Tensor conv1x1_wgrad(torch::Tensor dy, torch::Tensor x);
std::vector<torch::Tensor> conv3x3_fwd(torch::Tensor a, torch::Tensor w9,
                                       int64_t imgH, int64_t imgW,
                                       c10::optional<torch::Tensor> bias,
                                       c10::optional<torch::Tensor> scale,
                                       c10::optional<torch::Tensor> shift,
                                       c10::optional<torch::Tensor> residual,
                                       bool relu, bool want_stats);
torch::Tensor conv3x3_wgrad(torch::Tensor dy, torch::Tensor x, int64_t imgH,
                            int64_t imgW);
torch::Tensor dwconv_fwd(torch::Tensor x, torch::Tensor weight,
                         c10::optional<torch::Tensor> bias, int64_t stride);
torch::Tensor dwconv_dgrad(torch::Tensor dy, torch::Tensor weight, int64_t H,
                           int64_t W, int64_t stride);
std::vector<torch::Tensor> dwconv_wgrad(torch::Tensor dy, torch::Tensor x,
                                        int64_t K, int64_t stride,
                                        bool out_f32);
torch::Tensor transpose2d(torch::Tensor src);
torch::Tensor stride2_gather(torch::Tensor x);
torch::Tensor stride2_scatter(torch::Tensor dy, int64_t IH, int64_t IW);
std::vector<torch::Tensor> softmax_ce_fwd(torch::Tensor logits,
                                          c10::optional<torch::Tensor> target,
                                          c10::optional<torch::Tensor> soft_target,
                                          double smoothing, int64_t ignore_index);
torch::Tensor softmax_ce_bwd(torch::Tensor logits,
                             c10::optional<torch::Tensor> target,
                             c10::optional<torch::Tensor> soft_target,
                             torch::Tensor lse, double smoothing,
                             int64_t ignore_index, torch::Tensor grad_out,
                             torch::Tensor stats);
torch::Tensor focal_loss_fwd(torch::Tensor logits, torch::Tensor targets,
                             double alpha, double gamma);
torch::Tensor focal_loss_bwd(torch::Tensor dloss, torch::Tensor logits,
                             torch::Tensor targets, double alpha, double gamma);
torch::Tensor box_iou_gpu(torch::Tensor a, torch::Tensor b, bool giou);
torch::Tensor nms_gpu(torch::Tensor boxes_sorted, double iou_threshold);
torch::Tensor roialign_fwd(torch::Tensor input, torch::Tensor rois, int64_t PH,
                           int64_t PW, double spatial_scale,
                           int64_t sampling_ratio, bool aligned);
torch::Tensor roialign_bwd(torch::Tensor grad_out, torch::Tensor rois, int64_t N,
                           int64_t C, int64_t H, int64_t W, double spatial_scale,
                           int64_t sampling_ratio, bool aligned);
std::vector<torch::Tensor> attn_fwd(torch::Tensor qkv, int64_t num_heads,
                                    double scale,
                                    c10::optional<torch::Tensor> bias,
                                    c10::optional<torch::Tensor> mask,
                                    bool save_p, bool save_stats);
std::vector<torch::Tensor> attn_bwd(torch::Tensor qkv, torch::Tensor dout,
                                    torch::Tensor stats, torch::Tensor drow,
                                    int64_t num_heads, double scale);
std::vector<torch::Tensor> attn_fwd_cosine(torch::Tensor qkv, int64_t num_heads,
                              torch::Tensor logit_scale,
                              c10::optional<torch::Tensor> bias,
                              c10::optional<torch::Tensor> mask, bool save_p);
torch::Tensor mfma_probe(torch::Tensor A, torch::Tensor B);
torch::Tensor my_add(torch::Tensor a, torch::Tensor b);
std::vector<torch::Tensor> cocoeval_match_image(
    torch::Tensor det_boxes, torch::Tensor det_scores, torch::Tensor gt_boxes,
    torch::Tensor gt_crowd, torch::Tensor iou_thrs, int64_t max_dets,
    c10::optional<torch::Tensor> gt_extra_ignore);
torch::Tensor window_partition_fwd(torch::Tensor x, int64_t ws, int64_t shift);
torch::Tensor window_partition_bwd(torch::Tensor grad, int64_t B, int64_t H,
                                   int64_t W, int64_t ws, int64_t shift);
torch::Tensor window_merge_fwd(torch::Tensor windows, int64_t B, int64_t H,
                               int64_t W, int64_t ws, int64_t shift);
torch::Tensor window_merge_bwd(torch::Tensor grad, int64_t ws, int64_t shift);

PYBIND11_MODULE(TORCH_EXTENSION_NAME, m) {
  m.doc() = "deeplearning_amd gfx950 HIP kernels";
  m.def("layernorm_fwd", &layernorm_fwd);
  m.def("layernorm_bwd", &layernorm_bwd);
  m.def("gelu_fwd", &gelu_fwd);
  m.def("gelu_bwd", &gelu_bwd);
  m.def("silu_fwd", &silu_fwd);
  m.def("silu_bwd", &silu_bwd);
  m.def("add_relu_fwd", &add_relu_fwd);
  m.def("relu_mask_bwd", &relu_mask_bwd);
  m.def("batchnorm_fwd", &batchnorm_fwd);
  m.def("batchnorm_fwd_from_sums", &batchnorm_fwd_from_sums);
  m.def("bn_apply", &bn_apply);
  m.def("batchnorm_bwd", &batchnorm_bwd);
  m.def("batchnorm_bwd_ex", &batchnorm_bwd_ex);
  m.def("bn_relu_mask_from_x", &bn_relu_mask_from_x);
  m.def("bn_relu_maxpool_fwd", &bn_relu_maxpool_fwd);
  m.def("bn_relu_maxpool_bwd", &bn_relu_maxpool_bwd);
  m.def("bn_add_relu_fwd_from_sums", &bn_add_relu_fwd_from_sums);
  m.def("bn_add_relu_dual_fwd_from_sums", &bn_add_relu_dual_fwd_from_sums);
  m.def("bn_add_relu_bwd", &bn_add_relu_bwd);
  m.def("bn_add_relu_dual_bwd", &bn_add_relu_dual_bwd);
  m.def("conv1x1_fwd", &conv1x1_fwd, py::arg("a"), py::arg("b"),
        py::arg("bias") = py::none(), py::arg("scale") = py::none(),
        py::arg("shift") = py::none(), py::arg("residual") = py::none(),
        py::arg("relu") = false, py::arg("want_stats") = false);
  m.def("conv1x1_dgrad_bwdstats", &conv1x1_dgrad_bwdstats, py::arg("dy"),
        py::arg("wt"), py::arg("residual"), py::arg("mode"), py::arg("out"),
        py::arg("x"), py::arg("scale"), py::arg("shift"), py::arg("mean"),
        py::arg("rstd"), py::arg("xd") = py::none(),
        py::arg("mean_d") = py::none(), py::arg("rstd_d") = py::none());
  m.def("bn_slab_reduce", &bn_slab_reduce);
  m.def("bn_bwd_dx_from_slab", &bn_bwd_dx_from_slab);
  m.def("bn_join_dual_bwd_dx_from_slab", &bn_join_dual_bwd_dx_from_slab);
  m.def("conv1x1_wgrad", &conv1x1_wgrad);
  m.def("conv3x3_fwd", &conv3x3_fwd, py::arg("a"), py::arg("w9"),
        py::arg("imgH"), py::arg("imgW"), py::arg("bias") = py::none(),
        py::arg("scale") = py::none(), py::arg("shift") = py::none(),
        py::arg("residual") = py::none(), py::arg("relu") = false,
        py::arg("want_stats") = false);
  m.def("conv3x3_wgrad", &conv3x3_wgrad);
  m.def("dwconv_fwd", &dwconv_fwd, py::arg("x"), py::arg("weight"),
        py::arg("bias") = py::none(), py::arg("stride") = 1);
  m.def("dwconv_dgrad", &dwconv_dgrad);
  m.def("dwconv_wgrad", &dwconv_wgrad);
  m.def("transpose2d", &transpose2d);
  m.def("stride2_gather", &stride2_gather);
  m.def("stride2_scatter", &stride2_scatter);
  m.def("softmax_ce_fwd", &softmax_ce_fwd);
  m.def("softmax_ce_bwd", &softmax_ce_bwd);
  m.def("focal_loss_fwd", &focal_loss_fwd);
  m.def("focal_loss_bwd", &focal_loss_bwd);
  m.def("box_iou", &box_iou_gpu);
  m.def("nms", &nms_gpu);
  m.def("roialign_fwd", &roialign_fwd);
  m.def("roialign_bwd", &roialign_bwd);
  m.def("attn_fwd", &attn_fwd, py::arg("qkv"), py::arg("num_heads"),
        py::arg("scale"), py::arg("bias") = py::none(),
        py::arg("mask") = py::none(), py::arg("save_p") = false,
        py::arg("save_stats") = false);
  m.def("attn_bwd", &attn_bwd);
  m.def("attn_fwd_cosine", &attn_fwd_cosine, py::arg("qkv"),
        py::arg("num_heads"), py::arg("logit_scale"),
        py::arg("bias") = py::none(), py::arg("mask") = py::none(),
        py::arg("save_p") = false);
  m.def("mfma_probe", &mfma_probe);
  m.def("cocoeval_match_image", &cocoeval_match_image, py::arg("det_boxes"),
        py::arg("det_scores"), py::arg("gt_boxes"), py::arg("gt_crowd"),
        py::arg("iou_thrs"), py::arg("max_dets"),
        py::arg("gt_extra_ignore") = py::none());
  m.def("my_add", &my_add);
  m.def("window_partition_fwd", &window_partition_fwd);
  m.def("window_partition_bwd", &window_partition_bwd);
  m.def("window_merge_fwd", &window_merge_fwd);
  m.def("window_merge_bwd", &window_merge_bwd);
}
```

csrc/reorder.hip:

```cpp
#include "common.h"
#include "vec.h"

namespace dla {

using bf16 = __hip_bfloat16;

inline int64_t nhwc_used_threads_pub(int lanes_per_row, int64_t rows,
                                     int64_t target_lanes) {
  int64_t k = target_lanes / lanes_per_row;
  if (k > rows) k = rows;
  if (k < 1) k = 1;
  return (int64_t)lanes_per_row * k;
}

__global__ __launch_bounds__(256) void transpose2d_kernel(
    const bf16* __restrict__ src, bf16* __restrict__ dst, int R, int C) {
  __shared__ bf16 tile[32][33];
  const int tx = threadIdx.x & 31, ty = threadIdx.x >> 5;
  const int c0 = blockIdx.x * 32, r0 = blockIdx.y * 32;
#pragma unroll
  for (int i = 0; i < 4; ++i) {
    const int r = r0 + ty + i * 8;
    const int c = c0 + tx;
    if (r < R && c < C) tile[ty + i * 8][tx] = src[(int64_t)r * C + c];
  }
  __syncthreads();
#pragma unroll
  for (int i = 0; i < 4; ++i) {
    const int r = c0 + ty + i * 8;
    const int c = r0 + tx;
    if (r < C && c < R) dst[(int64_t)r * R + c] = tile[tx][ty + i * 8];
  }
}


template <typename dev_t, int V>
__global__ void stride2_gather_kernel(const dev_t* __restrict__ src,
                                      dev_t* __restrict__ dst, int C, int IH,
                                      int IW, int OH, int OW, int64_t M_out,
                                      int64_t used) {
  const int64_t t = (int64_t)blockIdx.x * blockDim.x + threadIdx.x;
  if (t >= used) return;
  const int lanes = C / V;
  const int c0 = (int)(t % lanes) * V;
  const int64_t rstride = used / lanes;
  for (int64_t m = t / lanes; m < M_out; m += rstride) {
    const int64_t bo = m / ((int64_t)OH * OW);
    const int64_t r = m - bo * OH * OW;
    const int oh = (int)(r / OW), ow = (int)(r % OW);
    const int64_t src_row = (bo * (int64_t)IH + oh * 2) * IW + ow * 2;
    vstore<dev_t, V>(dst + m * C + c0,
                     vload<dev_t, V>(src + src_row * C + c0));
  }
}

template <typename dev_t, int V>
__global__ void stride2_scatter_kernel(const dev_t* __restrict__ src,
                                       dev_t* __restrict__ dst, int C, int IH,
                                       int IW, int OH, int OW, int64_t M_in,
                                       int64_t used) {
  const int64_t t = (int64_t)blockIdx.x * blockDim.x + threadIdx.x;
  if (t >= used) return;
  const int lanes = C / V;
  const int c0 = (int)(t % lanes) * V;
  const int64_t rstride = used / lanes;
  for (int64_t m = t / lanes; m < M_in; m += rstride) {
    const int64_t bi = m / ((int64_t)IH * IW);
    const int64_t r = m - bi * IH * IW;
    const int ih = (int)(r / IW), iw = (int)(r % IW);
    Vec<dev_t, V> v;
    if ((ih & 1) == 0 && (iw & 1) == 0) {
      const int64_t src_row =
          (bi * (int64_t)OH + (ih >> 1)) * OW + (iw >> 1);
      v = vload<dev_t, V>(src + src_row * C + c0);
    } else {
#pragma unroll
      for (int j = 0; j < V; ++j) v.v[j] = from_f32<dev_t>(0.f);
    }
    vstore<dev_t, V>(dst + m * C + c0, v);
  }
}

}

torch::Tensor transpose2d(torch::Tensor src) {
  DLA_CHECK_INPUT(src);
  TORCH_CHECK(src.dim() == 2 && src.scalar_type() == torch::kBFloat16,
              "transpose2d: 2D bf16");
  const int R = (int)src.size(0), C = (int)src.size(1);
  auto dst = torch::empty({C, R}, src.options());
  hipLaunchKernelGGL(dla::transpose2d_kernel,
                     dim3((C + 31) / 32, (R + 31) / 32), dim3(256), 0,
                     dla::stream(), (const dla::bf16*)src.data_ptr(),
                     (dla::bf16*)dst.data_ptr(), R, C);
  HIP_CHECK_ERR();
  return dst;
}

torch::Tensor stride2_gather(torch::Tensor x) {
  DLA_CHECK_CUDA(x);
  TORCH_CHECK(x.dim() == 4, "stride2_gather: 4D");
  TORCH_CHECK(x.is_contiguous(at::MemoryFormat::ChannelsLast),
              "stride2_gather: channels_last");
  const int B = (int)x.size(0), C = (int)x.size(1);
  const int IH = (int)x.size(2), IW = (int)x.size(3);
  const int OH = (IH + 1) / 2, OW = (IW + 1) / 2;
  auto y = torch::empty({B, C, OH, OW},
                        x.options().memory_format(at::MemoryFormat::ChannelsLast));
  const int64_t M_out = (int64_t)B * OH * OW;
  DLA_DISPATCH_FLOAT_TYPES(x.scalar_type(), "stride2_gather", [&] {
    constexpr int VM = 16 / (int)sizeof(dev_t);
    const int V = (C % VM == 0) ? VM : 1;
    auto run = [&](auto vtag) {
      constexpr int VV = decltype(vtag)::value;
      const int lanes = C / VV;
      const int64_t used = dla::nhwc_used_threads_pub(lanes, M_out, 262144);
      hipLaunchKernelGGL((dla::stride2_gather_kernel<dev_t, VV>),
                         dim3((unsigned)((used + 255) / 256)),
                         dim3(256), 0, dla::stream(),
                         (const dev_t*)x.data_ptr(), (dev_t*)y.data_ptr(), C,
                         IH, IW, OH, OW, M_out, used);
    };
    if (V == VM) run(std::integral_constant<int, VM>{});
    else run(std::integral_constant<int, 1>{});
  });
  HIP_CHECK_ERR();
  return y;
}

torch::Tensor stride2_scatter(torch::Tensor dy, int64_t IH, int64_t IW) {
  DLA_CHECK_CUDA(dy);
  TORCH_CHECK(dy.dim() == 4, "stride2_scatter: 4D");
  TORCH_CHECK(dy.is_contiguous(at::MemoryFormat::ChannelsLast),
              "stride2_scatter: channels_last");
  const int B = (int)dy.size(0), C = (int)dy.size(1);
  const int OH = (int)dy.size(2), OW = (int)dy.size(3);
  auto dx = torch::empty({B, C, IH, IW},
                         dy.options().memory_format(at::MemoryFormat::ChannelsLast));
  const int64_t M_in = (int64_t)B * IH * IW;
  DLA_DISPATCH_FLOAT_TYPES(dy.scalar_type(), "stride2_scatter", [&] {
    constexpr int VM = 16 / (int)sizeof(dev_t);
    auto run = [&](auto vtag) {
      constexpr int VV = decltype(vtag)::value;
      const int lanes = C / VV;
      const int64_t used = dla::nhwc_used_threads_pub(lanes, M_in, 524288);
      hipLaunchKernelGGL((dla::stride2_scatter_kernel<dev_t, VV>),
                         dim3((unsigned)((used + 255) / 256)), dim3(256), 0,
                         dla::stream(), (const dev_t*)dy.data_ptr(),
                         (dev_t*)dx.data_ptr(), C, (int)IH, (int)IW, OH, OW,
                         M_in, used);
    };
    if (C % VM == 0) run(std::integral_constant<int, VM>{});
    else run(std::integral_constant<int, 1>{});
  });
  HIP_CHECK_ERR();
  return dx;
}
```

deeplearning_amd/models/classification/resnet.py:

```python
from __future__ import annotations

import torch
import torch.nn as nn

from ...ops import BatchNorm2d, add_relu, bn_relu_maxpool
from ...ops.conv1x1 import (can_pass_input, conv1x1_bn, conv_bn,
                            conv_bn_add_relu)
from ..registry import register_model


def _downsample_fwd(downsample, x):
    if (isinstance(downsample, nn.Sequential) and len(downsample) == 2 and
            isinstance(downsample[0], nn.Conv2d)):
        return conv_bn(x, downsample[0], downsample[1])
    return downsample(x)


class _NormRelu(nn.Sequential):

    def __init__(self, norm, c):
        super().__init__(norm(c), nn.ReLU(inplace=True))


def make_norm(norm_layer, c, relu=False):
    if not relu:
        return norm_layer(c)
    try:
        return norm_layer(c, relu=True)
    except TypeError:
        return _NormRelu(norm_layer, c)


def conv3x3(cin, cout, stride=1, groups=1, dilation=1):
    return nn.Conv2d(cin, cout, 3, stride=stride, padding=dilation, groups=groups,
                     bias=False, dilation=dilation)


def conv1x1(cin, cout, stride=1):
    return nn.Conv2d(cin, cout, 1, stride=stride, bias=False)


class BasicBlock(nn.Module):
    expansion = 1

    def __init__(self, inplanes, planes, stride=1, downsample=None, groups=1,
                 base_width=64, dilation=1, norm_layer=None):
        super().__init__()
        norm_layer = norm_layer or BatchNorm2d
        if groups != 1 or base_width != 64:
            raise ValueError("BasicBlock only supports groups=1, base_width=64")
        self.conv1 = conv3x3(inplanes, planes, stride)
        self.bn1 = make_norm(norm_layer, planes, relu=True)
        self.conv2 = conv3x3(planes, planes)
        self.bn2 = norm_layer(planes)
        self.downsample = downsample
        self.stride = stride

    def forward(self, x):
        identity = x
        out = conv_bn(x, self.conv1, self.bn1)
        out = conv_bn(out, self.conv2, self.bn2)
        if self.downsample is not None:
            identity = _downsample_fwd(self.downsample, x)
        return add_relu(out, identity)


class Bottleneck(nn.Module):
    expansion = 4

    def __init__(self, inplanes, planes, stride=1, downsample=None, groups=1,
                 base_width=64, dilation=1, norm_layer=None):
        super().__init__()
        norm_layer = norm_layer or BatchNorm2d
        width = int(planes * (base_width / 64.0)) * groups
        self.conv1 = conv1x1(inplanes, width)
        self.bn1 = make_norm(norm_layer, width, relu=True)
        self.conv2 = conv3x3(width, width, stride, groups, dilation)
        self.bn2 = make_norm(norm_layer, width, relu=True)
        self.conv3 = conv1x1(width, planes * self.expansion)
        self.bn3 = norm_layer(planes * self.expansion)
        self.downsample = downsample
        self.stride = stride

    def forward(self, x):
        identity = x
        if self.downsample is None and can_pass_input(x, self.conv1, self.bn1):
            out, identity = conv1x1_bn(x, self.conv1, self.bn1,
                                       pass_input=True)
        else:
            out = conv_bn(x, self.conv1, self.bn1)
        out = conv_bn(out, self.conv2, self.bn2)
        return conv_bn_add_relu(out, self.conv3, self.bn3, identity=identity,
                                x_down=x, downsample=self.downsample)


class ResNet(nn.Module):
    def __init__(self, block, layers, num_classes=1000, groups=1, width_per_group=64,
                 replace_stride_with_dilation=None, norm_layer=None,
                 zero_init_residual=False, include_top=True):
        super().__init__()
        self._norm_layer = norm_layer or BatchNorm2d
        self.inplanes = 64
        self.dilation = 1
        replace_stride_with_dilation = replace_stride_with_dilation or [False] * 3
        self.groups = groups
        self.base_width = width_per_group
        self.include_top = include_top

        self.conv1 = nn.Conv2d(3, 64, 7, stride=2, padding=3, bias=False)
        self.bn1 = make_norm(self._norm_layer, 64, relu=True)
        self.maxpool = nn.MaxPool2d(3, stride=2, padding=1)
        self.layer1 = self._make_layer(block, 64, layers[0])
        self.layer2 = self._make_layer(block, 128, layers[1], stride=2,
                                       dilate=replace_stride_with_dilation[0])
        self.layer3 = self._make_layer(block, 256, layers[2], stride=2,
                                       dilate=replace_stride_with_dilation[1])
        self.layer4 = self._make_layer(block, 512, layers[3], stride=2,
                                       dilate=replace_stride_with_dilation[2])
        if include_top:
            self.avgpool = nn.AdaptiveAvgPool2d(1)
            self.fc = nn.Linear(512 * block.expansion, num_classes)

        for m in self.modules():
            if isinstance(m, nn.Conv2d):
                nn.init.kaiming_normal_(m.weight, mode="fan_out", nonlinearity="relu")
            elif isinstance(m, (nn.BatchNorm2d, nn.GroupNorm)):
                nn.init.ones_(m.weight)
                nn.init.zeros_(m.bias)
        if zero_init_residual:
            for m in self.modules():
                if isinstance(m, Bottleneck):
                    nn.init.zeros_(m.bn3.weight)
                elif isinstance(m, BasicBlock):
                    nn.init.zeros_(m.bn2.weight)

    def _make_layer(self, block, planes, blocks, stride=1, dilate=False):
        norm_layer = self._norm_layer
        downsample = None
        prev_dilation = self.dilation
        if dilate:
            self.dilation *= stride
            stride = 1
        if stride != 1 or self.inplanes != planes * block.expansion:
            downsample = nn.Sequential(
                conv1x1(self.inplanes, planes * block.expansion, stride),
                norm_layer(planes * block.expansion),
            )
        layers = [block(self.inplanes, planes, stride, downsample, self.groups,
                        self.base_width, prev_dilation, norm_layer)]
        self.inplanes = planes * block.expansion
        for _ in range(1, blocks):
            layers.append(block(self.inplanes, planes, groups=self.groups,
                                base_width=self.base_width, dilation=self.dilation,
                                norm_layer=norm_layer))
        return nn.Sequential(*layers)

    def forward_features(self, x):
        x = bn_relu_maxpool(self.conv1(x), self.bn1, self.maxpool)
        x = self.layer1(x)
        x = self.layer2(x)
        x = self.layer3(x)
        x = self.layer4(x)
        return x

    def forward(self, x):
        x = self.forward_features(x)
        if self.include_top:
            x = self.avgpool(x)
            x = torch.flatten(x, 1)
            x = self.fc(x)
        return x


@register_model
def resnet18(num_classes=1000, **kw):
    return ResNet(BasicBlock, [2, 2, 2, 2], num_classes=num_classes, **kw)


@register_model
def resnet34(num_classes=1000, **kw):
    return ResNet(BasicBlock, [3, 4, 6, 3], num_classes=num_classes, **kw)


@register_model
def resnet50(num_classes=1000, **kw):
    return ResNet(Bottleneck, [3, 4, 6, 3], num_classes=num_classes, **kw)


@register_model
def resnet101(num_classes=1000, **kw):
    return ResNet(Bottleneck, [3, 4, 23, 3], num_classes=num_classes, **kw)


@register_model
def resnet152(num_classes=1000, **kw):
    return ResNet(Bottleneck, [3, 8, 36, 3], num_classes=num_classes, **kw)


@register_model
def resnext50_32x4d(num_classes=1000, **kw):
    return ResNet(Bottleneck, [3, 4, 6, 3], num_classes=num_classes, groups=32,
                  width_per_group=4, **kw)


@register_model
def resnext101_32x8d(num_classes=1000, **kw):
    return ResNet(Bottleneck, [3, 4, 23, 3], num_classes=num_classes, groups=32,
                  width_per_group=8, **kw)


@register_model
def wide_resnet50_2(num_classes=1000, **kw):
    return ResNet(Bottleneck, [3, 4, 6, 3], num_classes=num_classes,
                  width_per_group=128, **kw)


@register_model
def wide_resnet101_2(num_classes=1000, **kw):
    return ResNet(Bottleneck, [3, 4, 23, 3], num_classes=num_classes,
                  width_per_group=128, **kw)
```

deeplearning_amd/ops/batchnorm.py:

```python
from __future__ import annotations

import os

import torch
import torch.nn as nn
import torch.nn.functional as F

from ._ext import dense, ext, use_hip


def _mask_from_y() -> bool:
    return os.environ.get("DLA_BN_MASK_FROM_Y", "0") == "1"


def save_bn_for_backward(ctx, x, y, weight, mean, rstd, scale, shift, relu):
    ctx.relu = relu
    ctx.mask_from_x = bool(relu and not _mask_from_y() and
                           ext().bn_relu_mask_from_x(x))
    if ctx.mask_from_x:
        ctx.save_for_backward(x, weight, mean, rstd, scale, shift)
    elif relu:
        ctx.save_for_backward(x, weight, mean, rstd, y)
    else:
        ctx.save_for_backward(x, weight, mean, rstd)


RELU_X, JOIN, JOIN_DUAL = 1, 2, 3


def bwd_stats_epilogue_disabled() -> bool:
    return (os.environ.get("DLA_NO_BWD_STATS_EPILOGUE", "0") == "1" or
            os.environ.get("DLA_NO_FUSED_JOIN", "0") == "1")


class BwdStatsLink:

    __slots__ = ("mode", "operands", "g", "slab", "g_version")

    def __init__(self, mode, **operands):
        self.mode = mode
        self.operands = operands
        self.g = self.slab = self.g_version = None

    def take_operands(self):
        ops, self.operands = self.operands, None
        return ops

    def offer(self, g, slab):
        self.g, self.slab, self.g_version = g, slab, g._version

    def claim(self, dy, like):
        g, slab, version = self.g, self.slab, self.g_version
        self.g = self.slab = self.g_version = None
        if g is None or dy is None or not dy.is_cuda:
            return None
        same = (dy.dtype == g.dtype and dy.shape == like.shape and
                dy.stride() == like.stride() and dy.storage_offset() == 0 and
                dy.data_ptr() == g.data_ptr() and
                dy.untyped_storage().data_ptr() ==
                g.untyped_storage().data_ptr() and dy._version == version)
        return slab if same else None


def link_eligible(x) -> bool:
    return (x.is_cuda and x.dtype == torch.bfloat16 and x.dim() == 4 and
            x.shape[1] % 64 == 0 and
            x.is_contiguous(memory_format=torch.channels_last))


def relu_x_epilogue_enabled() -> bool:
    return os.environ.get("DLA_BWD_STATS_RELU_X", "0") == "1"


def attach_relu_link(y):
    fn = y.grad_fn
    if fn is None or not getattr(fn, "mask_from_x", False) or \
            not relu_x_epilogue_enabled() or bwd_stats_epilogue_disabled():
        return y
    x, _, mean, rstd, scale, shift = fn.saved_tensors
    if link_eligible(x):
        fn.link = y._dla_bwd_link = BwdStatsLink(
            RELU_X, x_raw=x, mean=mean, rstd=rstd, scale=scale, shift=shift)
    return y


def bn_backward(ctx, dy):
    x, weight, mean, rstd, *rest = ctx.saved_tensors
    link = getattr(ctx, "link", None)
    if link is not None:
        slab = link.claim(dy, x)
        if slab is not None:
            return ext().bn_bwd_dx_from_slab(dy, slab, x, weight, mean, rstd)
    y = scale = shift = None
    if ctx.mask_from_x:
        scale, shift = rest
    elif ctx.relu:
        y, = rest
    return ext().batchnorm_bwd_ex(dy, x, y, weight, mean, rstd, scale, shift,
                                  ctx.relu)


class _BNFn(torch.autograd.Function):
    @staticmethod
    def forward(ctx, x, weight, bias, running_mean, running_var, momentum, eps, relu):
        x = dense(x)
        y, mean, rstd, scale, shift = ext().batchnorm_fwd(
            x, weight, bias, running_mean, running_var, momentum, eps, relu)
        save_bn_for_backward(ctx, x, y, weight, mean, rstd, scale, shift, relu)
        return y

    @staticmethod
    def backward(ctx, dy):
        dx, dw, db = bn_backward(ctx, dy)
        return dx, dw, db, None, None, None, None, None


class BatchNorm2d(nn.BatchNorm2d):

    def __init__(self, num_features, eps=1e-5, momentum=0.1, relu=False):
        super().__init__(num_features, eps=eps, momentum=momentum, affine=True,
                         track_running_stats=True)
        self.relu = relu

    def _eaf(self) -> float:
        if self.momentum is not None:
            return self.momentum
        if self.training and self.num_batches_tracked is not None:
            return 1.0 / float(max(int(self.num_batches_tracked), 1))
        return 0.0

    def forward(self, x):
        if not use_hip(x):
            if self.training and self.momentum is None and \
                    self.num_batches_tracked is not None:
                self.num_batches_tracked.add_(1)
            y = F.batch_norm(x, self.running_mean, self.running_var, self.weight,
                             self.bias, self.training, self._eaf(), self.eps)
            return torch.relu(y) if self.relu else y
        if self.running_mean.dtype != torch.float32:
            self.running_mean.data = self.running_mean.data.float()
            self.running_var.data = self.running_var.data.float()
        if self.training:
            if self.num_batches_tracked is not None:
                self.num_batches_tracked.add_(1)
            y = _BNFn.apply(x, self.weight, self.bias, self.running_mean,
                            self.running_var, self._eaf(), self.eps,
                            self.relu)
            return attach_relu_link(y) if self.relu else y
        rstd = torch.rsqrt(self.running_var.float() + self.eps)
        scale = self.weight.float() * rstd
        shift = self.bias.float() - self.running_mean.float() * scale
        if torch.is_grad_enabled() and (x.requires_grad or self.weight.requires_grad):
            y = x * scale.reshape(1, -1, 1, 1).to(x.dtype) + shift.reshape(1, -1, 1, 1).to(x.dtype)
            return torch.relu(y) if self.relu else y
        return ext().bn_apply(dense(x), scale, shift, self.relu)


class FrozenBatchNorm2d(nn.Module):

    def __init__(self, num_features, eps=1e-5):
        super().__init__()
        self.eps = eps
        self.register_buffer("weight", torch.ones(num_features))
        self.register_buffer("bias", torch.zeros(num_features))
        self.register_buffer("running_mean", torch.zeros(num_features))
        self.register_buffer("running_var", torch.ones(num_features))

    def _load_from_state_dict(self, state_dict, prefix, *args, **kwargs):
        state_dict.pop(prefix + "num_batches_tracked", None)
        super()._load_from_state_dict(state_dict, prefix, *args, **kwargs)

    def forward(self, x):
        rstd = torch.rsqrt(self.running_var.float() + self.eps)
        scale = self.weight.float() * rstd
        shift = self.bias.float() - self.running_mean.float() * scale
        if use_hip(x) and not (torch.is_grad_enabled() and x.requires_grad):
            return ext().bn_apply(dense(x), scale, shift, False)
        sc = scale.reshape(1, -1, 1, 1).to(x.dtype)
        sh = shift.reshape(1, -1, 1, 1).to(x.dtype)
        return x * sc + sh
```

deeplearning_amd/ops/conv1x1.py:

```python
from __future__ import annotations

import os

import torch
import torch.nn.functional as F
from torch import nn

from ._ext import ext, use_hip
from .batchnorm import (JOIN, JOIN_DUAL, RELU_X, BwdStatsLink,
                        attach_relu_link, bn_backward,
                        bwd_stats_epilogue_disabled, link_eligible,
                        save_bn_for_backward)


def _flatten_nhwc(x: torch.Tensor) -> torch.Tensor:
    B, C, H, W = x.shape
    return x.permute(0, 2, 3, 1).reshape(B * H * W, C)


def _unflatten_nhwc(y2d: torch.Tensor, B: int, H: int, W: int) -> torch.Tensor:
    return y2d.view(B, H, W, -1).permute(0, 3, 1, 2)


class _Conv1x1Fn(torch.autograd.Function):

    @staticmethod
    def forward(ctx, x2d, w, bias, scale, shift, residual, relu, want_stats,
                pass_input=False, link=None):
        xb = x2d if x2d.dtype == torch.bfloat16 else x2d.to(torch.bfloat16)
        ctx.link = link if xb is x2d else None
        wb = w if w.dtype == torch.bfloat16 else w.to(torch.bfloat16)
        wb = wb.contiguous()
        y2d, sums = ext().conv1x1_fwd(xb, wb, bias, scale, shift, residual,
                                      relu, want_stats)
        ctx.save_for_backward(xb, wb)
        ctx.x_dtype = x2d.dtype
        ctx.w_dtype = w.dtype
        ctx.pass_input = pass_input
        outs = (y2d,)
        if want_stats:
            ctx.mark_non_differentiable(sums)
            outs += (sums,)
        if pass_input:
            ctx.set_materialize_grads(False)
            outs += (x2d,)
        return outs if len(outs) > 1 else y2d

    @staticmethod
    def backward(ctx, dy2d, *rest):
        xb, wb = ctx.saved_tensors
        d_alias = rest[-1] if ctx.pass_input else None
        if d_alias is not None:
            d_alias = d_alias.contiguous()
        dx = dw = db = None
        if dy2d is None:
            if d_alias is not None and ctx.needs_input_grad[0]:
                dx = d_alias.to(ctx.x_dtype)
            return dx, None, None, None, None, None, None, None, None, None
        dy2d = dy2d.contiguous()
        if dy2d.dtype != torch.bfloat16:
            dy2d = dy2d.to(torch.bfloat16)
        if ctx.needs_input_grad[0]:
            wt = ext().transpose2d(wb)
            if d_alias is not None and d_alias.dtype != torch.bfloat16:
                d_alias = d_alias.to(torch.bfloat16)
            link = ctx.link
            ops = link.take_operands() if link is not None else None
            if ops is not None and ops["x_raw"].numel() == xb.numel() and \
                    ops["x_raw"].shape[1] == xb.shape[1]:
                dx, slab = ext().conv1x1_dgrad_bwdstats(
                    dy2d, wt, d_alias, link.mode,
                    None if link.mode == RELU_X else xb, ops["x_raw"],
                    ops.get("scale"), ops.get("shift"), ops["mean"],
                    ops["rstd"], ops.get("xd_raw"), ops.get("mean_d"),
                    ops.get("rstd_d"))
                link.offer(dx, slab)
            else:
                dx, _ = ext().conv1x1_fwd(dy2d, wt, None, None, None,
                                          d_alias, False, False)
            if dx.dtype != ctx.x_dtype:
                dx = dx.to(ctx.x_dtype)
        if ctx.needs_input_grad[1]:
            dw = ext().conv1x1_wgrad(dy2d, xb)
            if dw.dtype != ctx.w_dtype:
                dw = dw.to(ctx.w_dtype)
        if ctx.needs_input_grad[2]:
            db = dy2d.float().sum(0)
        return dx, dw, db, None, None, None, None, None, None, None


class _BNFromStatsFn(torch.autograd.Function):

    @staticmethod
    def forward(ctx, x, weight, bias, sums, running_mean, running_var,
                momentum, eps, relu):
        y, mean, rstd, scale, shift = ext().batchnorm_fwd_from_sums(
            x, weight, bias, sums, running_mean, running_var, momentum, eps,
            relu)
        save_bn_for_backward(ctx, x, y, weight, mean, rstd, scale, shift,
                             relu)
        return y

    @staticmethod
    def backward(ctx, dy):
        dx, dw, db = bn_backward(ctx, dy)
        return dx, dw, db, None, None, None, None, None, None


class _Stride2Fn(torch.autograd.Function):

    @staticmethod
    def forward(ctx, x):
        ctx.ihw = (x.shape[2], x.shape[3])
        return ext().stride2_gather(x)

    @staticmethod
    def backward(ctx, dy):
        if not dy.is_contiguous(memory_format=torch.channels_last):
            dy = dy.contiguous(memory_format=torch.channels_last)
        return ext().stride2_scatter(dy, *ctx.ihw)


def _conv1x1_disabled() -> bool:
    return os.environ.get("DLA_NO_CONV1X1", "0") == "1"


def can_fuse_conv1x1(x: torch.Tensor, conv: nn.Conv2d) -> bool:
    if _conv1x1_disabled() or not use_hip(x):
        return False
    if x.dtype != torch.bfloat16:
        return False
    if conv.kernel_size != (1, 1) or conv.groups != 1:
        return False
    if conv.padding != (0, 0) or conv.dilation != (1, 1):
        return False
    if conv.stride not in ((1, 1), (2, 2)):
        return False
    cin, cout = conv.in_channels, conv.out_channels
    if cin % 64 != 0 or cout % 64 != 0:
        return False
    return x.dim() == 4 and x.is_contiguous(memory_format=torch.channels_last)


def _prep(x: torch.Tensor, conv: nn.Conv2d):
    stride = conv.stride[0]
    if stride == 2:
        x = _Stride2Fn.apply(x)
    B, C, H, W = x.shape
    x2d = _flatten_nhwc(x)
    w2d = conv.weight.reshape(conv.weight.shape[0], conv.weight.shape[1])
    bias = conv.bias.float() if conv.bias is not None else None
    return x2d, w2d, bias, (B, H, W)


def conv1x1(x: torch.Tensor, conv: nn.Conv2d) -> torch.Tensor:
    x2d, wb, bias, (B, H, W) = _prep(x, conv)
    y2d = _Conv1x1Fn.apply(x2d, wb, bias, None, None, None, False, False)
    return _unflatten_nhwc(y2d, B, H, W)


def _fp32_running_stats(bn) -> None:
    if bn.running_mean.dtype != torch.float32:
        bn.running_mean.data = bn.running_mean.data.float()
        bn.running_var.data = bn.running_var.data.float()


def _conv1x1_train_stats(x: torch.Tensor, conv: nn.Conv2d, bn,
                         pass_input: bool = False):
    link = getattr(x, "_dla_bwd_link", None)
    if link is not None and (
            bwd_stats_epilogue_disabled() or conv.stride != (1, 1) or
            x.dtype != torch.bfloat16 or
            (link.mode != RELU_X and not pass_input)):
        link = None
    x2d, wb, bias, (B, H, W) = _prep(x, conv)
    _fp32_running_stats(bn)
    if bn.num_batches_tracked is not None:
        bn.num_batches_tracked.add_(1)
    momentum = bn._eaf() if hasattr(bn, "_eaf") else (bn.momentum or 0.0)
    outs = _Conv1x1Fn.apply(x2d, wb, bias, None, None, None, False, True,
                            pass_input, link)
    alias = _unflatten_nhwc(outs[2], B, H, W) if pass_input else None
    return _unflatten_nhwc(outs[0], B, H, W), outs[1], momentum, alias


def conv1x1_bn(x: torch.Tensor, conv: nn.Conv2d, bn,
               pass_input: bool = False):
    relu = bool(getattr(bn, "relu", False))
    if bn.training:
        y_raw, partials, momentum, alias = _conv1x1_train_stats(
            x, conv, bn, pass_input)
        y = _BNFromStatsFn.apply(y_raw, bn.weight, bn.bias, partials,
                                 bn.running_mean, bn.running_var, momentum,
                                 bn.eps, relu)
        if relu:
            attach_relu_link(y)
        return (y, alias) if pass_input else y
    if pass_input:
        raise ValueError("conv1x1_bn: pass_input needs train mode")

    x2d, wb, bias, (B, H, W) = _prep(x, conv)
    _fp32_running_stats(bn)

    if not bn.training:
        rstd = torch.rsqrt(bn.running_var + bn.eps)
        scale = bn.weight.float() * rstd
        shift = bn.bias.float() - bn.running_mean * scale
        if not (torch.is_grad_enabled() and
                (x.requires_grad or conv.weight.requires_grad or
                 bn.weight.requires_grad)):
            y2d, _ = ext().conv1x1_fwd(
                x2d.to(torch.bfloat16), wb.to(torch.bfloat16).contiguous(),
                bias, scale.contiguous(), shift.contiguous(), None, relu,
                False)
            return _unflatten_nhwc(y2d, B, H, W)
        y2d = _Conv1x1Fn.apply(x2d, wb, bias, None, None, None, False, False)
        y = _unflatten_nhwc(y2d, B, H, W)
        y = y * scale.reshape(1, -1, 1, 1).to(y.dtype) + \
            shift.reshape(1, -1, 1, 1).to(y.dtype)
        return torch.relu(y) if relu else y


class _BNJoinFn(torch.autograd.Function):

    @staticmethod
    def forward(ctx, x_raw, weight, bias, partials, running_mean,
                running_var, momentum, eps, identity):
        out, mean, rstd = ext().bn_add_relu_fwd_from_sums(
            x_raw, weight, bias, partials, running_mean, running_var,
            momentum, eps, identity)
        ctx.save_for_backward(x_raw, out, weight, mean, rstd)
        return out

    @staticmethod
    def backward(ctx, dy):
        x_raw, out, weight, mean, rstd = ctx.saved_tensors
        link = getattr(ctx, "link", None)
        slab = link.claim(dy, out) if link is not None else None
        if slab is not None:
            g = dy
            dx, dw, db = ext().bn_bwd_dx_from_slab(g, slab, x_raw, weight,
                                                   mean, rstd)
        else:
            g, dx, dw, db = ext().bn_add_relu_bwd(dy, out, x_raw, weight,
                                                  mean, rstd)
        return dx, dw, db, None, None, None, None, None, g


class _BNJoinDualFn(torch.autograd.Function):

    @staticmethod
    def forward(ctx, x_raw, weight, bias, partials, running_mean,
                running_var, momentum, eps, xd_raw, weight_d, bias_d,
                partials_d, running_mean_d, running_var_d, momentum_d, eps_d):
        out, mean, rstd, mean_d, rstd_d = \
            ext().bn_add_relu_dual_fwd_from_sums(
                x_raw, weight, bias, partials, running_mean, running_var,
                momentum, eps, xd_raw, weight_d, bias_d, partials_d,
                running_mean_d, running_var_d, momentum_d, eps_d)
        ctx.save_for_backward(x_raw, xd_raw, out, weight, mean, rstd,
                              weight_d, mean_d, rstd_d)
        return out

    @staticmethod
    def backward(ctx, dy):
        (x_raw, xd_raw, out, weight, mean, rstd, weight_d, mean_d,
         rstd_d) = ctx.saved_tensors
        link = getattr(ctx, "link", None)
        slab = link.claim(dy, out) if link is not None else None
        if slab is not None:
            dx, dxd, dw, db, dwd, dbd = \
                ext().bn_join_dual_bwd_dx_from_slab(
                    dy, slab, x_raw, weight, mean, rstd, xd_raw, weight_d,
                    mean_d, rstd_d)
        else:
            dx, dxd, dw, db, dwd, dbd = ext().bn_add_relu_dual_bwd(
                dy, out, x_raw, weight, mean, rstd, xd_raw, weight_d,
                mean_d, rstd_d)
        return (dx, dw, db, None, None, None, None, None,
                dxd, dwd, dbd, None, None, None, None, None)


def _fused_join_disabled() -> bool:
    return os.environ.get("DLA_NO_FUSED_JOIN", "0") == "1"


def _dual_epilogue_disabled() -> bool:
    return os.environ.get("DLA_NO_BWD_STATS_DUAL", "0") == "1"


def _attach_join_link(out: torch.Tensor) -> torch.Tensor:
    fn = out.grad_fn
    if fn is None or bwd_stats_epilogue_disabled():
        return out
    saved = fn.saved_tensors
    if len(saved) == 5:
        x_raw, _, _, mean, rstd = saved
        if link_eligible(x_raw):
            fn.link = out._dla_bwd_link = BwdStatsLink(
                JOIN, x_raw=x_raw, mean=mean, rstd=rstd)
    elif not _dual_epilogue_disabled():
        x_raw, xd_raw, _, _, mean, rstd, _, mean_d, rstd_d = saved
        if link_eligible(x_raw):
            fn.link = out._dla_bwd_link = BwdStatsLink(
                JOIN_DUAL, x_raw=x_raw, mean=mean, rstd=rstd, xd_raw=xd_raw,
                mean_d=mean_d, rstd_d=rstd_d)
    return out


def _join_bn_ok(conv: nn.Conv2d, bn) -> bool:
    from .batchnorm import BatchNorm2d

    return (type(bn) is BatchNorm2d and bn.training and
            not getattr(bn, "relu", False) and conv.bias is None)


def can_pass_input(x: torch.Tensor, conv: nn.Conv2d, bn) -> bool:
    from .batchnorm import BatchNorm2d

    return (not _fused_join_disabled() and can_fuse_conv1x1(x, conv) and
            conv.stride == (1, 1) and type(bn) is BatchNorm2d and
            bn.training and torch.is_grad_enabled() and x.requires_grad)


def can_fuse_join(x: torch.Tensor, conv: nn.Conv2d, bn, identity=None,
                  x_down=None, downsample=None) -> bool:
    if _fused_join_disabled() or not can_fuse_conv1x1(x, conv) or \
            not _join_bn_ok(conv, bn):
        return False
    if downsample is not None:
        if not (isinstance(downsample, nn.Sequential) and
                len(downsample) == 2 and
                isinstance(downsample[0], nn.Conv2d)):
            return False
        return (x_down is not None and
                can_fuse_conv1x1(x_down, downsample[0]) and
                _join_bn_ok(downsample[0], downsample[1]) and
                downsample[0].out_channels == conv.out_channels)
    return (identity is not None and use_hip(identity) and
            identity.dtype == torch.bfloat16 and identity.dim() == 4 and
            identity.is_contiguous(memory_format=torch.channels_last))


def conv_bn_add_relu(x: torch.Tensor, conv: nn.Conv2d, bn, identity=None,
                     x_down=None, downsample=None) -> torch.Tensor:
    if can_fuse_join(x, conv, bn, identity, x_down, downsample):
        y_raw, partials, momentum, _ = _conv1x1_train_stats(x, conv, bn)
        if downsample is None:
            if identity.shape != y_raw.shape:
                raise ValueError("conv_bn_add_relu: identity shape mismatch")
            return _attach_join_link(_BNJoinFn.apply(
                y_raw, bn.weight, bn.bias, partials, bn.running_mean,
                bn.running_var, momentum, bn.eps, identity))
        conv_d, bn_d = downsample[0], downsample[1]
        yd_raw, partials_d, momentum_d, _ = _conv1x1_train_stats(
            x_down, conv_d, bn_d)
        if yd_raw.shape != y_raw.shape:
            raise ValueError("conv_bn_add_relu: downsample shape mismatch")
        return _attach_join_link(_BNJoinDualFn.apply(
            y_raw, bn.weight, bn.bias, partials, bn.running_mean,
            bn.running_var, momentum, bn.eps, yd_raw, bn_d.weight, bn_d.bias,
            partials_d, bn_d.running_mean, bn_d.running_var, momentum_d,
            bn_d.eps))
    from .activations import add_relu

    out = conv_bn(x, conv, bn)
    if downsample is not None:
        if (isinstance(downsample, nn.Sequential) and len(downsample) == 2
                and isinstance(downsample[0], nn.Conv2d)):
            identity = conv_bn(x_down, downsample[0], downsample[1])
        else:
            identity = downsample(x_down)
    return add_relu(out, identity)


def conv_bn(x: torch.Tensor, conv: nn.Conv2d, bn) -> torch.Tensor:
    from .batchnorm import BatchNorm2d

    if isinstance(bn, BatchNorm2d):
        if can_fuse_conv1x1(x, conv):
            return conv1x1_bn(x, conv, bn)
        if can_fuse_conv3x3(x, conv):
            return conv3x3_bn(x, conv, bn)
    return bn(conv(x))


class _Conv3x3Fn(torch.autograd.Function):

    @staticmethod
    def forward(ctx, x4d, w, want_stats):
        B, C, H, W = x4d.shape
        xb = x4d if x4d.dtype == torch.bfloat16 else x4d.to(torch.bfloat16)
        wb = w if w.dtype == torch.bfloat16 else w.to(torch.bfloat16)
        a = _flatten_nhwc(xb)
        w9 = wb.permute(0, 2, 3, 1).reshape(w.shape[0], -1).contiguous()
        y2d, sums = ext().conv3x3_fwd(a, w9, H, W, None, None, None, None,
                                      False, want_stats)
        ctx.save_for_backward(xb, wb)
        ctx.w_dtype = w.dtype
        ctx.x_dtype = x4d.dtype
        y = _unflatten_nhwc(y2d, B, H, W)
        if want_stats:
            ctx.mark_non_differentiable(sums)
            return y, sums
        return y

    @staticmethod
    def backward(ctx, dy, *unused):
        xb, wb = ctx.saved_tensors
        B, C, H, W = xb.shape
        if not dy.is_contiguous(memory_format=torch.channels_last):
            dy = dy.contiguous(memory_format=torch.channels_last)
        if dy.dtype != torch.bfloat16:
            dy = dy.to(torch.bfloat16)
        dy2d = _flatten_nhwc(dy)
        dx = dw = None
        if ctx.needs_input_grad[0]:
            wd = wb.flip(2, 3).transpose(0, 1)
            wd9 = wd.permute(0, 2, 3, 1).reshape(C, -1).contiguous()
            dx2d, _ = ext().conv3x3_fwd(dy2d, wd9, H, W, None, None, None,
                                        None, False, False)
            dx = _unflatten_nhwc(dx2d, B, H, W)
            if dx.dtype != ctx.x_dtype:
                dx = dx.to(ctx.x_dtype)
        if ctx.needs_input_grad[1]:
            dw9 = ext().conv3x3_wgrad(dy2d, _flatten_nhwc(xb), H, W)
            dw = dw9.view(wb.shape[0], 3, 3, C).permute(0, 3, 1, 2)
            if dw.dtype != ctx.w_dtype:
                dw = dw.to(ctx.w_dtype)
            else:
                dw = dw.contiguous()
        return dx, dw, None


def _conv3x3_enabled() -> bool:
    return os.environ.get("DLA_CONV3X3", "0") == "1"


def can_fuse_conv3x3(x: torch.Tensor, conv: nn.Conv2d) -> bool:
    if _conv1x1_disabled() or not _conv3x3_enabled() or not use_hip(x):
        return False
    if x.dtype != torch.bfloat16:
        return False
    if conv.kernel_size != (3, 3) or conv.groups != 1:
        return False
    if conv.padding != (1, 1) or conv.dilation != (1, 1) or \
            conv.stride != (1, 1) or conv.bias is not None:
        return False
    if conv.in_channels % 64 != 0 or conv.out_channels % 64 != 0:
        return False
    return x.dim() == 4 and x.is_contiguous(memory_format=torch.channels_last)


def conv3x3_bn(x: torch.Tensor, conv: nn.Conv2d, bn) -> torch.Tensor:
    relu = bool(getattr(bn, "relu", False))
    B, C, H, W = x.shape
    if bn.running_mean.dtype != torch.float32:
        bn.running_mean.data = bn.running_mean.data.float()
        bn.running_var.data = bn.running_var.data.float()
    if not bn.training:
        rstd = torch.rsqrt(bn.running_var + bn.eps)
        scale = bn.weight.float() * rstd
        shift = bn.bias.float() - bn.running_mean * scale
        if not (torch.is_grad_enabled() and
                (x.requires_grad or conv.weight.requires_grad or
                 bn.weight.requires_grad)):
            xb = x.to(torch.bfloat16)
            wb = conv.weight.to(torch.bfloat16)
            w9 = wb.permute(0, 2, 3, 1).reshape(wb.shape[0], -1).contiguous()
            y2d, _ = ext().conv3x3_fwd(_flatten_nhwc(xb), w9, H, W, None,
                                       scale.contiguous(), shift.contiguous(),
                                       None, relu, False)
            return _unflatten_nhwc(y2d, B, H, W)
        y = _Conv3x3Fn.apply(x, conv.weight, False)
        y = y * scale.reshape(1, -1, 1, 1).to(y.dtype) + \
            shift.reshape(1, -1, 1, 1).to(y.dtype)
        return torch.relu(y) if relu else y
    if bn.num_batches_tracked is not None:
        bn.num_batches_tracked.add_(1)
    momentum = bn._eaf() if hasattr(bn, "_eaf") else (bn.momentum or 0.0)
    y_raw, partials = _Conv3x3Fn.apply(x, conv.weight, True)
    return _BNFromStatsFn.apply(y_raw, bn.weight, bn.bias, partials,
                                bn.running_mean, bn.running_var, momentum,
                                bn.eps, relu)
```

deeplearning_amd/ops/stem.py:

```python
from __future__ import annotations

import os

import torch
from torch import nn

from ._ext import ext, use_hip


class _BNReluMaxPoolFn(torch.autograd.Function):
    @staticmethod
    def forward(ctx, x, weight, bias, running_mean, running_var, momentum,
                eps):
        pooled, slots, mean, rstd, scale, shift = ext().bn_relu_maxpool_fwd(
            x, weight, bias, running_mean, running_var, momentum, eps)
        ctx.save_for_backward(x, slots, weight, mean, rstd, scale, shift)
        return pooled

    @staticmethod
    def backward(ctx, dpool):
        x, slots, weight, mean, rstd, scale, shift = ctx.saved_tensors
        dx, dw, db = ext().bn_relu_maxpool_bwd(dpool, x, slots, weight, mean,
                                               rstd, scale, shift)
        return dx, dw, db, None, None, None, None


def _fused_stem_disabled() -> bool:
    return os.environ.get("DLA_NO_FUSED_STEM", "0") == "1"


def _pair(v):
    return tuple(v) if isinstance(v, (tuple, list)) else (v, v)


def can_fuse_stem(x: torch.Tensor, bn, pool) -> bool:
    from .batchnorm import BatchNorm2d

    if _fused_stem_disabled() or not use_hip(x):
        return False
    if type(bn) is not BatchNorm2d or not bn.relu or not bn.training:
        return False
    if type(pool) is not nn.MaxPool2d or pool.ceil_mode or \
            pool.return_indices:
        return False
    if (_pair(pool.kernel_size), _pair(pool.stride), _pair(pool.padding),
            _pair(pool.dilation)) != ((3, 3), (2, 2), (1, 1), (1, 1)):
        return False
    if x.dtype not in (torch.bfloat16, torch.float16, torch.float32):
        return False
    if x.dim() != 4 or x.numel() == 0 or \
            x.shape[1] % (16 // x.element_size()) != 0:
        return False
    if x.shape[0] * x.shape[2] * x.shape[3] >= 2 ** 31:
        return False
    return x.is_contiguous(memory_format=torch.channels_last) and \
        not x.is_contiguous()


def bn_relu_maxpool(x: torch.Tensor, bn, pool) -> torch.Tensor:
    if not can_fuse_stem(x, bn, pool):
        return pool(bn(x))
    if bn.running_mean.dtype != torch.float32:
        bn.running_mean.data = bn.running_mean.data.float()
        bn.running_var.data = bn.running_var.data.float()
    if bn.num_batches_tracked is not None:
        bn.num_batches_tracked.add_(1)
    return _BNReluMaxPoolFn.apply(x, bn.weight, bn.bias, bn.running_mean,
                                  bn.running_var, bn._eaf(), bn.eps)
```

Baseline: 10070 images/s.

## Fold BN batch counter increment into finalize kernels and add packed bf16 weight arena

Removes the separate num_batches_tracked.add_(1) launch per BatchNorm layer by passing the counter pointer into the finalize kernels, where one thread increments it. The change also adds weight_pack_table and weight_pack_bf16 ops so conv weights can be pre-packed into a bf16 arena instead of being cast on every call. Together these cut small kernel launches and per-step host overhead across ResNet-50's many BN and conv layers. The cost is wider kernel signatures, plus a new code path for keeping packed weights current after updates.

```diff
diff --git a/csrc/batchnorm.hip b/csrc/batchnorm.hip
--- a/csrc/batchnorm.hip
+++ b/csrc/batchnorm.hip
@@ -47,6 +47,11 @@
   shift[c] = bias[c] - mu * sc;
 }
 
+__device__ __forceinline__ void bn_count_batch(int64_t* num_batches) {
+  if (num_batches != nullptr && blockIdx.x == 0 && threadIdx.x == 0)
+    *num_batches += 1;
+}
+
 __global__ void bn_finalize_kernel(const float* __restrict__ sums,
                                    const float* __restrict__ weight,
                                    const float* __restrict__ bias,
@@ -54,8 +59,10 @@
                                    float* __restrict__ running_mean,
                                    float* __restrict__ running_var,
                                    float* __restrict__ scale, float* __restrict__ shift,
-                                   int C, float count, float eps, float momentum) {
+                                   int C, float count, float eps, float momentum,
+                                   int64_t* __restrict__ num_batches) {
   const int c = blockIdx.x * blockDim.x + threadIdx.x;
+  bn_count_batch(num_batches);
   if (c >= C) return;
   bn_finalize_channel(c, sums[c], sums[C + c], weight, bias, mean, rstd,
                       running_mean, running_var, scale, shift, count, eps,
@@ -72,8 +79,10 @@
                          float* __restrict__ running_mean,
                          float* __restrict__ running_var,
                          float* __restrict__ scale, float* __restrict__ shift,
-                         int C, float count, float eps, float momentum) {
+                         int C, float count, float eps, float momentum,
+                         int64_t* __restrict__ num_batches) {
   __shared__ float ls[2][kFinRows][kFinCh + 1];
+  bn_count_batch(num_batches);
   const int cl = threadIdx.x % kFinCh, rl = threadIdx.x / kFinCh;
   const int c = blockIdx.x * kFinCh + cl;
   float s = 0.f, q = 0.f;
@@ -622,11 +631,22 @@
   torch::Tensor mean, rstd, scale, shift;
 };
 
+inline int64_t* bn_counter_ptr(const c10::optional<torch::Tensor>& num_batches,
+                               const torch::Tensor& like) {
+  if (!num_batches.has_value()) return nullptr;
+  TORCH_CHECK(num_batches->is_cuda() && num_batches->device() == like.device() &&
+                  num_batches->scalar_type() == torch::kLong &&
+                  num_batches->numel() == 1,
+              "num_batches_tracked must be one int64 on the input's device");
+  return num_batches->data_ptr<int64_t>();
+}
+
 inline BnFinalized bn_finalize_launch(
     const torch::Tensor& sums, const torch::Tensor& weight,
     const torch::Tensor& bias, c10::optional<torch::Tensor>& running_mean,
     c10::optional<torch::Tensor>& running_var, int C, int64_t rows,
-    double momentum, double eps) {
+    double momentum, double eps,
+    const c10::optional<torch::Tensor>& num_batches = c10::nullopt) {
   TORCH_CHECK(sums.is_cuda() && sums.scalar_type() == torch::kFloat &&
                   sums.is_contiguous(),
               "bn sums must be a contiguous fp32 GPU tensor");
@@ -643,6 +663,7 @@
   auto b32 = bias.to(torch::kFloat).contiguous();
   float* rm = running_mean.has_value() ? running_mean->data_ptr<float>() : nullptr;
   float* rv = running_var.has_value() ? running_var->data_ptr<float>() : nullptr;
+  int64_t* nb = bn_counter_ptr(num_batches, sums);
   const int n_parts = sums.dim() == 2 ? (int)sums.size(0) : 1;
   if (n_parts > 1) {
     hipLaunchKernelGGL(bn_finalize_parts_kernel, dim3((C + kFinCh - 1) / kFinCh),
@@ -651,14 +672,14 @@
                        b32.data_ptr<float>(), f.mean.data_ptr<float>(),
                        f.rstd.data_ptr<float>(), rm, rv,
                        f.scale.data_ptr<float>(), f.shift.data_ptr<float>(), C,
-                       (float)rows, (float)eps, (float)momentum);
+                       (float)rows, (float)eps, (float)momentum, nb);
   } else {
     hipLaunchKernelGGL(bn_finalize_kernel, dim3((C + 255) / 256), dim3(256), 0,
                        stream(), sums.data_ptr<float>(), w32.data_ptr<float>(),
                        b32.data_ptr<float>(), f.mean.data_ptr<float>(),
                        f.rstd.data_ptr<float>(), rm, rv,
                        f.scale.data_ptr<float>(), f.shift.data_ptr<float>(), C,
-                       (float)rows, (float)eps, (float)momentum);
+                       (float)rows, (float)eps, (float)momentum, nb);
   }
   return f;
 }
@@ -699,9 +720,11 @@
                                          torch::Tensor bias,
                                          c10::optional<torch::Tensor> running_mean,
                                          c10::optional<torch::Tensor> running_var,
-                                         double momentum, double eps, bool relu) {
+                                         double momentum, double eps, bool relu,
+                                         c10::optional<torch::Tensor> num_batches) {
   DLA_CHECK_CUDA(x);
   TORCH_CHECK(x.dim() == 4, "batchnorm_fwd expects a 4D tensor");
+  int64_t* nb = dla::bn_counter_ptr(num_batches, x);
   const bool nhwc = dla::is_nhwc(x);
   TORCH_CHECK(nhwc || x.is_contiguous(), "batchnorm_fwd: x must be contiguous "
               "(NCHW or channels_last)");
@@ -750,14 +773,14 @@
                          w32.data_ptr<float>(), b32.data_ptr<float>(),
                          mean.data_ptr<float>(), rstd.data_ptr<float>(), rm, rv,
                          scale.data_ptr<float>(), shift.data_ptr<float>(), C,
-                         (float)rows, (float)eps, (float)momentum);
+                         (float)rows, (float)eps, (float)momentum, nb);
     } else {
       hipLaunchKernelGGL(dla::bn_finalize_kernel, dim3((C + 255) / 256), dim3(256), 0,
                          dla::stream(), sums.data_ptr<float>(), w32.data_ptr<float>(),
                          b32.data_ptr<float>(), mean.data_ptr<float>(),
                          rstd.data_ptr<float>(), rm, rv,
                          scale.data_ptr<float>(), shift.data_ptr<float>(), C,
-                         (float)rows, (float)eps, (float)momentum);
+                         (float)rows, (float)eps, (float)momentum, nb);
     }
     const int64_t n_total = x.numel();
     constexpr int VMAX = 16 / (int)sizeof(dev_t);
@@ -799,7 +822,7 @@
     torch::Tensor x, torch::Tensor weight, torch::Tensor bias,
     torch::Tensor sums, c10::optional<torch::Tensor> running_mean,
     c10::optional<torch::Tensor> running_var, double momentum, double eps,
-    bool relu) {
+    bool relu, c10::optional<torch::Tensor> num_batches) {
   DLA_CHECK_CUDA(x);
   TORCH_CHECK(x.dim() == 4, "batchnorm_fwd_from_sums expects a 4D tensor");
   const bool nhwc = dla::is_nhwc(x);
@@ -810,7 +833,8 @@
   auto y = torch::empty_like(x);
   const int64_t rows = (int64_t)N * HW;
   auto fin = dla::bn_finalize_launch(sums, weight, bias, running_mean,
-                                     running_var, C, rows, momentum, eps);
+                                     running_var, C, rows, momentum, eps,
+                                     num_batches);
   auto& mean = fin.mean;
   auto& rstd = fin.rstd;
   auto& scale = fin.scale;
@@ -1039,7 +1063,7 @@
     torch::Tensor x, torch::Tensor weight, torch::Tensor bias,
     torch::Tensor sums, c10::optional<torch::Tensor> running_mean,
     c10::optional<torch::Tensor> running_var, double momentum, double eps,
-    torch::Tensor identity) {
+    torch::Tensor identity, c10::optional<torch::Tensor> num_batches) {
   DLA_CHECK_CUDA(x);
   TORCH_CHECK(dla::is_nhwc_rows(x), "bn_add_relu: x must be channels_last");
   dla::join_check(x, identity, "identity");
@@ -1047,7 +1071,8 @@
   const int C = (int)x.size(1);
   const int64_t rows = x.numel() / C;
   auto fin = dla::bn_finalize_launch(sums, weight, bias, running_mean,
-                                     running_var, C, rows, momentum, eps);
+                                     running_var, C, rows, momentum, eps,
+                                     num_batches);
   auto out = torch::empty_like(x);
   DLA_DISPATCH_FLOAT_TYPES(x.scalar_type(), "bn_add_relu_fwd_from_sums", [&] {
     constexpr int V = 16 / (int)sizeof(dev_t);
@@ -1070,7 +1095,8 @@
     torch::Tensor xd, torch::Tensor weight_d, torch::Tensor bias_d,
     torch::Tensor sums_d, c10::optional<torch::Tensor> running_mean_d,
     c10::optional<torch::Tensor> running_var_d, double momentum_d,
-    double eps_d) {
+    double eps_d, c10::optional<torch::Tensor> num_batches,
+    c10::optional<torch::Tensor> num_batches_d) {
   DLA_CHECK_CUDA(x);
   TORCH_CHECK(dla::is_nhwc_rows(x), "bn_add_relu_dual: x must be channels_last");
   dla::join_check(x, xd, "xd");
@@ -1078,9 +1104,11 @@
   const int C = (int)x.size(1);
   const int64_t rows = x.numel() / C;
   auto fin = dla::bn_finalize_launch(sums, weight, bias, running_mean,
-                                     running_var, C, rows, momentum, eps);
+                                     running_var, C, rows, momentum, eps,
+                                     num_batches);
   auto fd = dla::bn_finalize_launch(sums_d, weight_d, bias_d, running_mean_d,
-                                    running_var_d, C, rows, momentum_d, eps_d);
+                                    running_var_d, C, rows, momentum_d, eps_d,
+                                    num_batches_d);
   auto out = torch::empty_like(x);
   DLA_DISPATCH_FLOAT_TYPES(x.scalar_type(), "bn_add_relu_dual_fwd_from_sums", [&] {
     constexpr int V = 16 / (int)sizeof(dev_t);
@@ -1489,7 +1517,8 @@
 std::vector<torch::Tensor> bn_relu_maxpool_fwd(
     torch::Tensor x, torch::Tensor weight, torch::Tensor bias,
     c10::optional<torch::Tensor> running_mean,
-    c10::optional<torch::Tensor> running_var, double momentum, double eps) {
+    c10::optional<torch::Tensor> running_var, double momentum, double eps,
+    c10::optional<torch::Tensor> num_batches) {
   dla::stem_check(x, "bn_relu_maxpool_fwd");
   const int N = (int)x.size(0), C = (int)x.size(1);
   const int H = (int)x.size(2), W = (int)x.size(3);
@@ -1512,7 +1541,8 @@
                        dla::stream(), (const dev_t*)x.data_ptr(),
                        sums.data_ptr<float>(), C, rows, t.bl, t.rb);
     fin = dla::bn_finalize_launch(sums, weight, bias, running_mean,
-                                  running_var, C, rows, momentum, eps);
+                                  running_var, C, rows, momentum, eps,
+                                  num_batches);
     hipLaunchKernelGGL((dla::bn_relu_maxpool_fwd_nhwc_kernel<dev_t, V>),
                        dim3(N * runs), dim3(256), 0, dla::stream(),
                        (const dev_t*)x.data_ptr(), fin.scale.data_ptr<float>(),
diff --git a/csrc/bindings.cpp b/csrc/bindings.cpp
--- a/csrc/bindings.cpp
+++ b/csrc/bindings.cpp
@@ -15,7 +15,8 @@
                                          torch::Tensor bias,
                                          c10::optional<torch::Tensor> running_mean,
                                          c10::optional<torch::Tensor> running_var,
-                                         double momentum, double eps, bool relu);
+                                         double momentum, double eps, bool relu,
+                                         c10::optional<torch::Tensor> num_batches);
 torch::Tensor bn_apply(torch::Tensor x, torch::Tensor scale, torch::Tensor shift,
                        bool relu);
 std::vector<torch::Tensor> batchnorm_bwd(torch::Tensor dy, torch::Tensor x,
@@ -31,7 +32,8 @@
 std::vector<torch::Tensor> bn_relu_maxpool_fwd(
     torch::Tensor x, torch::Tensor weight, torch::Tensor bias,
     c10::optional<torch::Tensor> running_mean,
-    c10::optional<torch::Tensor> running_var, double momentum, double eps);
+    c10::optional<torch::Tensor> running_var, double momentum, double eps,
+    c10::optional<torch::Tensor> num_batches);
 std::vector<torch::Tensor> bn_relu_maxpool_bwd(
     torch::Tensor dpool, torch::Tensor x, torch::Tensor slots,
     torch::Tensor weight, torch::Tensor mean, torch::Tensor rstd,
@@ -40,12 +42,12 @@
     torch::Tensor x, torch::Tensor weight, torch::Tensor bias,
     torch::Tensor sums, c10::optional<torch::Tensor> running_mean,
     c10::optional<torch::Tensor> running_var, double momentum, double eps,
-    bool relu);
+    bool relu, c10::optional<torch::Tensor> num_batches);
 std::vector<torch::Tensor> bn_add_relu_fwd_from_sums(
     torch::Tensor x, torch::Tensor weight, torch::Tensor bias,
     torch::Tensor sums, c10::optional<torch::Tensor> running_mean,
     c10::optional<torch::Tensor> running_var, double momentum, double eps,
-    torch::Tensor identity);
+    torch::Tensor identity, c10::optional<torch::Tensor> num_batches);
 std::vector<torch::Tensor> bn_add_relu_dual_fwd_from_sums(
     torch::Tensor x, torch::Tensor weight, torch::Tensor bias,
     torch::Tensor sums, c10::optional<torch::Tensor> running_mean,
@@ -53,7 +55,8 @@
     torch::Tensor xd, torch::Tensor weight_d, torch::Tensor bias_d,
     torch::Tensor sums_d, c10::optional<torch::Tensor> running_mean_d,
     c10::optional<torch::Tensor> running_var_d, double momentum_d,
-    double eps_d);
+    double eps_d, c10::optional<torch::Tensor> num_batches,
+    c10::optional<torch::Tensor> num_batches_d);
 std::vector<torch::Tensor> bn_add_relu_bwd(torch::Tensor dy, torch::Tensor out,
                                            torch::Tensor x, torch::Tensor weight,
                                            torch::Tensor mean,
@@ -103,6 +106,11 @@
                                         int64_t K, int64_t stride,
                                         bool out_f32);
 torch::Tensor transpose2d(torch::Tensor src);
+std::tuple<torch::Tensor, int64_t, int64_t> weight_pack_table(
+    std::vector<torch::Tensor> srcs, std::vector<int64_t> off_nk,
+    std::vector<int64_t> off_kn);
+void weight_pack_bf16(torch::Tensor table, int64_t tiles, int64_t need,
+                      torch::Tensor arena);
 torch::Tensor stride2_gather(torch::Tensor x);
 torch::Tensor stride2_scatter(torch::Tensor dy, int64_t IH, int64_t IW);
 std::vector<torch::Tensor> softmax_ce_fwd(torch::Tensor logits,
@@ -162,16 +170,36 @@
   m.def("silu_bwd", &silu_bwd);
   m.def("add_relu_fwd", &add_relu_fwd);
   m.def("relu_mask_bwd", &relu_mask_bwd);
-  m.def("batchnorm_fwd", &batchnorm_fwd);
-  m.def("batchnorm_fwd_from_sums", &batchnorm_fwd_from_sums);
+  m.def("batchnorm_fwd", &batchnorm_fwd, py::arg("x"), py::arg("weight"),
+        py::arg("bias"), py::arg("running_mean"), py::arg("running_var"),
+        py::arg("momentum"), py::arg("eps"), py::arg("relu"),
+        py::arg("num_batches") = py::none());
+  m.def("batchnorm_fwd_from_sums", &batchnorm_fwd_from_sums, py::arg("x"),
+        py::arg("weight"), py::arg("bias"), py::arg("sums"),
+        py::arg("running_mean"), py::arg("running_var"), py::arg("momentum"),
+        py::arg("eps"), py::arg("relu"), py::arg("num_batches") = py::none());
   m.def("bn_apply", &bn_apply);
   m.def("batchnorm_bwd", &batchnorm_bwd);
   m.def("batchnorm_bwd_ex", &batchnorm_bwd_ex);
   m.def("bn_relu_mask_from_x", &bn_relu_mask_from_x);
-  m.def("bn_relu_maxpool_fwd", &bn_relu_maxpool_fwd);
+  m.def("bn_relu_maxpool_fwd", &bn_relu_maxpool_fwd, py::arg("x"),
+        py::arg("weight"), py::arg("bias"), py::arg("running_mean"),
+        py::arg("running_var"), py::arg("momentum"), py::arg("eps"),
+        py::arg("num_batches") = py::none());
   m.def("bn_relu_maxpool_bwd", &bn_relu_maxpool_bwd);
-  m.def("bn_add_relu_fwd_from_sums", &bn_add_relu_fwd_from_sums);
-  m.def("bn_add_relu_dual_fwd_from_sums", &bn_add_relu_dual_fwd_from_sums);
+  m.def("bn_add_relu_fwd_from_sums", &bn_add_relu_fwd_from_sums, py::arg("x"),
+        py::arg("weight"), py::arg("bias"), py::arg("sums"),
+        py::arg("running_mean"), py::arg("running_var"), py::arg("momentum"),
+        py::arg("eps"), py::arg("identity"),
+        py::arg("num_batches") = py::none());
+  m.def("bn_add_relu_dual_fwd_from_sums", &bn_add_relu_dual_fwd_from_sums,
+        py::arg("x"), py::arg("weight"), py::arg("bias"), py::arg("sums"),
+        py::arg("running_mean"), py::arg("running_var"), py::arg("momentum"),
+        py::arg("eps"), py::arg("xd"), py::arg("weight_d"), py::arg("bias_d"),
+        py::arg("sums_d"), py::arg("running_mean_d"),
+        py::arg("running_var_d"), py::arg("momentum_d"), py::arg("eps_d"),
+        py::arg("num_batches") = py::none(),
+        py::arg("num_batches_d") = py::none());
   m.def("bn_add_relu_bwd", &bn_add_relu_bwd);
   m.def("bn_add_relu_dual_bwd", &bn_add_relu_dual_bwd);
   m.def("conv1x1_fwd", &conv1x1_fwd, py::arg("a"), py::arg("b"),
@@ -198,6 +226,8 @@
   m.def("dwconv_dgrad", &dwconv_dgrad);
   m.def("dwconv_wgrad", &dwconv_wgrad);
   m.def("transpose2d", &transpose2d);
+  m.def("weight_pack_table", &weight_pack_table);
+  m.def("weight_pack_bf16", &weight_pack_bf16);
   m.def("stride2_gather", &stride2_gather);
   m.def("stride2_scatter", &stride2_scatter);
   m.def("softmax_ce_fwd", &softmax_ce_fwd);
diff --git a/csrc/reorder.hip b/csrc/reorder.hip
--- a/csrc/reorder.hip
+++ b/csrc/reorder.hip
@@ -30,6 +30,72 @@
     const int r = c0 + ty + i * 8;
     const int c = r0 + tx;
     if (r < C && c < R) dst[(int64_t)r * R + c] = tile[tx][ty + i * 8];
+  }
+}
+
+constexpr int kPackTile = 64;
+constexpr int kPackCols = 8;
+constexpr int kPackLdsRow = kPackTile + 2;
+
+__device__ __forceinline__ uint32_t pack_bf16_bits(float f) {
+  const uint32_t u = __float_as_uint(f);
+  if ((u & 0x7fffffffu) > 0x7f800000u) return 0x7fc0u;
+  return (u + 0x7fffu + ((u >> 16) & 1u)) >> 16;
+}
+
+__global__ __launch_bounds__(256) void weight_pack_bf16_kernel(
+    const int64_t* __restrict__ table, int n_entries,
+    uint16_t* __restrict__ arena, int64_t arena_elems) {
+  __shared__ __attribute__((aligned(4))) uint16_t tile[kPackTile][kPackLdsRow];
+  const int b = blockIdx.x;
+  int lo = 0, hi = n_entries - 1;
+  while (lo < hi) {
+    const int mid = (lo + hi + 1) >> 1;
+    if (table[(int64_t)mid * kPackCols + 6] <= b) lo = mid;
+    else hi = mid - 1;
+  }
+  const int64_t* e = table + (int64_t)lo * kPackCols;
+  const int N = (int)e[1], K = (int)e[2];
+  const bool src_bf16 = e[3] != 0;
+  const int t = b - (int)e[6];
+  const int tk = K / kPackTile;
+  const int r0 = (t / tk) * kPackTile, c0 = (t % tk) * kPackTile;
+  if (r0 >= N || e[4] + (int64_t)N * K > arena_elems ||
+      e[5] + (int64_t)N * K > arena_elems)
+    return;
+
+  const int cx = (threadIdx.x & 15) * 4, ry = threadIdx.x >> 4;
+  uint16_t* dst_nk = arena + e[4];
+  uint16_t* dst_kn = arena + e[5];
+#pragma unroll
+  for (int i = 0; i < 4; ++i) {
+    const int r = ry + i * 16;
+    const int64_t at = (int64_t)(r0 + r) * K + c0 + cx;
+    uint32_t lo2, hi2;
+    if (src_bf16) {
+      const uint2 v = *reinterpret_cast<const uint2*>(
+          reinterpret_cast<const uint16_t*>(e[0]) + at);
+      lo2 = v.x;
+      hi2 = v.y;
+    } else {
+      const float4 v = *reinterpret_cast<const float4*>(
+          reinterpret_cast<const float*>(e[0]) + at);
+      lo2 = pack_bf16_bits(v.x) | (pack_bf16_bits(v.y) << 16);
+      hi2 = pack_bf16_bits(v.z) | (pack_bf16_bits(v.w) << 16);
+    }
+    *reinterpret_cast<uint2*>(dst_nk + at) = make_uint2(lo2, hi2);
+    uint32_t* row = reinterpret_cast<uint32_t*>(&tile[r][cx]);
+    row[0] = lo2;
+    row[1] = hi2;
+  }
+  __syncthreads();
+#pragma unroll
+  for (int i = 0; i < 4; ++i) {
+    const int k = ry + i * 16;
+    const uint32_t lo2 = tile[cx][k] | ((uint32_t)tile[cx + 1][k] << 16);
+    const uint32_t hi2 = tile[cx + 2][k] | ((uint32_t)tile[cx + 3][k] << 16);
+    *reinterpret_cast<uint2*>(dst_kn + (int64_t)(c0 + k) * N + r0 + cx) =
+        make_uint2(lo2, hi2);
   }
 }
 
@@ -95,6 +161,76 @@
                      (dla::bf16*)dst.data_ptr(), R, C);
   HIP_CHECK_ERR();
   return dst;
+}
+
+std::tuple<torch::Tensor, int64_t, int64_t> weight_pack_table(
+    std::vector<torch::Tensor> srcs, std::vector<int64_t> off_nk,
+    std::vector<int64_t> off_kn) {
+  const int64_t n = (int64_t)srcs.size();
+  TORCH_CHECK(n > 0 && (int64_t)off_nk.size() == n &&
+                  (int64_t)off_kn.size() == n,
+              "weight_pack_table: one offset pair per source");
+  auto host = torch::zeros({n, dla::kPackCols}, torch::kLong);
+  int64_t* h = host.data_ptr<int64_t>();
+  std::vector<std::pair<int64_t, int64_t>> ranges;
+  int64_t tiles = 0, need = 0;
+  for (int64_t i = 0; i < n; ++i) {
+    const auto& s = srcs[i];
+    DLA_CHECK_INPUT(s);
+    TORCH_CHECK(s.device() == srcs[0].device(),
+                "weight_pack_table: sources on one device");
+    TORCH_CHECK(s.dim() == 2 && (s.scalar_type() == torch::kFloat ||
+                                 s.scalar_type() == torch::kBFloat16),
+                "weight_pack_table: sources are 2D fp32 or bf16");
+    const int64_t N = s.size(0), K = s.size(1);
+    TORCH_CHECK(N > 0 && K > 0 && N % dla::kPackTile == 0 &&
+                    K % dla::kPackTile == 0 && N * K < (int64_t(1) << 31),
+                "weight_pack_table: N and K must be multiples of 64");
+    TORCH_CHECK((uintptr_t)s.data_ptr() % 16 == 0,
+                "weight_pack_table: source must be 16-byte aligned");
+    for (int64_t off : {off_nk[i], off_kn[i]}) {
+      TORCH_CHECK(off >= 0 && off % 8 == 0,
+                  "weight_pack_table: offsets must be multiples of 8");
+      ranges.emplace_back(off, off + N * K);
+      need = std::max(need, off + N * K);
+    }
+    h[0] = (int64_t)(uintptr_t)s.data_ptr();
+    h[1] = N;
+    h[2] = K;
+    h[3] = s.scalar_type() == torch::kBFloat16;
+    h[4] = off_nk[i];
+    h[5] = off_kn[i];
+    h[6] = tiles;
+    h += dla::kPackCols;
+    tiles += (N / dla::kPackTile) * (K / dla::kPackTile);
+  }
+  std::sort(ranges.begin(), ranges.end());
+  for (size_t i = 1; i < ranges.size(); ++i)
+    TORCH_CHECK(ranges[i - 1].second <= ranges[i].first,
+                "weight_pack_table: destination ranges overlap");
+  TORCH_CHECK(tiles < (int64_t(1) << 31), "weight_pack_table: too many tiles");
+  return {host.to(srcs[0].device()), tiles, need};
+}
+
+void weight_pack_bf16(torch::Tensor table, int64_t tiles, int64_t need,
+                      torch::Tensor arena) {
+  DLA_CHECK_INPUT(table);
+  DLA_CHECK_INPUT(arena);
+  TORCH_CHECK(table.scalar_type() == torch::kLong && table.dim() == 2 &&
+                  table.size(0) > 0 && table.size(1) == dla::kPackCols,
+              "weight_pack_bf16: table must come from weight_pack_table");
+  TORCH_CHECK(arena.scalar_type() == torch::kBFloat16 &&
+                  arena.device() == table.device() && arena.numel() >= need &&
+                  (uintptr_t)arena.data_ptr() % 16 == 0,
+              "weight_pack_bf16: arena must be bf16, on the table's device, "
+              "16-byte aligned and hold `need` elements");
+  TORCH_CHECK(tiles > 0 && tiles < (int64_t(1) << 31),
+              "weight_pack_bf16: tiles out of range");
+  hipLaunchKernelGGL(dla::weight_pack_bf16_kernel, dim3((unsigned)tiles),
+                     dim3(256), 0, dla::stream(),
+                     table.data_ptr<int64_t>(), (int)table.size(0),
+                     (uint16_t*)arena.data_ptr(), arena.numel());
+  HIP_CHECK_ERR();
 }
 
 torch::Tensor stride2_gather(torch::Tensor x) {
diff --git a/deeplearning_amd/models/classification/resnet.py b/deeplearning_amd/models/classification/resnet.py
--- a/deeplearning_amd/models/classification/resnet.py
+++ b/deeplearning_amd/models/classification/resnet.py
@@ -4,7 +4,8 @@
 import torch.nn as nn
 
 from ...ops import BatchNorm2d, add_relu, bn_relu_maxpool
-from ...ops.conv1x1 import (can_pass_input, conv1x1_bn, conv_bn,
+from ...ops._ext import use_hip
+from ...ops.conv1x1 import (WeightPack, can_pass_input, conv1x1_bn, conv_bn,
                             conv_bn_add_relu)
 from ..registry import register_model
 
@@ -156,6 +157,8 @@
         return nn.Sequential(*layers)
 
     def forward_features(self, x):
+        if use_hip(x):
+            WeightPack.attach(self)
         x = bn_relu_maxpool(self.conv1(x), self.bn1, self.maxpool)
         x = self.layer1(x)
         x = self.layer2(x)
diff --git a/deeplearning_amd/ops/batchnorm.py b/deeplearning_amd/ops/batchnorm.py
--- a/deeplearning_amd/ops/batchnorm.py
+++ b/deeplearning_amd/ops/batchnorm.py
@@ -100,19 +100,32 @@
                                   ctx.relu)
 
 
+def bn_count_batch(bn):
+    nbt = bn.num_batches_tracked
+    in_kernel = (nbt is not None and bn.momentum is not None and
+                 nbt.is_cuda and nbt.dtype == torch.int64 and
+                 nbt.numel() == 1)
+    if nbt is not None and not in_kernel:
+        nbt.add_(1)
+    momentum = bn._eaf() if hasattr(bn, "_eaf") else (bn.momentum or 0.0)
+    return momentum, (nbt if in_kernel else None)
+
+
 class _BNFn(torch.autograd.Function):
     @staticmethod
-    def forward(ctx, x, weight, bias, running_mean, running_var, momentum, eps, relu):
+    def forward(ctx, x, weight, bias, running_mean, running_var, momentum, eps,
+                relu, num_batches=None):
         x = dense(x)
         y, mean, rstd, scale, shift = ext().batchnorm_fwd(
-            x, weight, bias, running_mean, running_var, momentum, eps, relu)
+            x, weight, bias, running_mean, running_var, momentum, eps, relu,
+            num_batches)
         save_bn_for_backward(ctx, x, y, weight, mean, rstd, scale, shift, relu)
         return y
 
     @staticmethod
     def backward(ctx, dy):
         dx, dw, db = bn_backward(ctx, dy)
-        return dx, dw, db, None, None, None, None, None
+        return dx, dw, db, None, None, None, None, None, None
 
 
 class BatchNorm2d(nn.BatchNorm2d):
@@ -141,11 +154,10 @@
             self.running_mean.data = self.running_mean.data.float()
             self.running_var.data = self.running_var.data.float()
         if self.training:
-            if self.num_batches_tracked is not None:
-                self.num_batches_tracked.add_(1)
+            momentum, counter = bn_count_batch(self)
             y = _BNFn.apply(x, self.weight, self.bias, self.running_mean,
-                            self.running_var, self._eaf(), self.eps,
-                            self.relu)
+                            self.running_var, momentum, self.eps, self.relu,
+                            counter)
             return attach_relu_link(y) if self.relu else y
         rstd = torch.rsqrt(self.running_var.float() + self.eps)
         scale = self.weight.float() * rstd
diff --git a/deeplearning_amd/ops/conv1x1.py b/deeplearning_amd/ops/conv1x1.py
--- a/deeplearning_amd/ops/conv1x1.py
+++ b/deeplearning_amd/ops/conv1x1.py
@@ -1,6 +1,7 @@
 from __future__ import annotations
 
 import os
+import weakref
 
 import torch
 import torch.nn.functional as F
@@ -8,7 +9,7 @@
 
 from ._ext import ext, use_hip
 from .batchnorm import (JOIN, JOIN_DUAL, RELU_X, BwdStatsLink,
-                        attach_relu_link, bn_backward,
+                        attach_relu_link, bn_backward, bn_count_batch,
                         bwd_stats_epilogue_disabled, link_eligible,
                         save_bn_for_backward)
 
@@ -26,14 +27,21 @@
 
     @staticmethod
     def forward(ctx, x2d, w, bias, scale, shift, residual, relu, want_stats,
-                pass_input=False, link=None):
+                pass_input=False, link=None, packed=None):
         xb = x2d if x2d.dtype == torch.bfloat16 else x2d.to(torch.bfloat16)
         ctx.link = link if xb is x2d else None
-        wb = w if w.dtype == torch.bfloat16 else w.to(torch.bfloat16)
-        wb = wb.contiguous()
+        if packed is not None:
+            wb, wt = packed
+        else:
+            wb = w if w.dtype == torch.bfloat16 else w.to(torch.bfloat16)
+            wb = wb.contiguous()
         y2d, sums = ext().conv1x1_fwd(xb, wb, bias, scale, shift, residual,
                                       relu, want_stats)
-        ctx.save_for_backward(xb, wb)
+        ctx.packed = packed is not None
+        if ctx.packed:
+            ctx.save_for_backward(xb, wb, wt)
+        else:
+            ctx.save_for_backward(xb, wb)
         ctx.x_dtype = x2d.dtype
         ctx.w_dtype = w.dtype
         ctx.pass_input = pass_input
@@ -48,7 +56,7 @@
 
     @staticmethod
     def backward(ctx, dy2d, *rest):
-        xb, wb = ctx.saved_tensors
+        xb, wb, *wt = ctx.saved_tensors
         d_alias = rest[-1] if ctx.pass_input else None
         if d_alias is not None:
             d_alias = d_alias.contiguous()
@@ -56,12 +64,12 @@
         if dy2d is None:
             if d_alias is not None and ctx.needs_input_grad[0]:
                 dx = d_alias.to(ctx.x_dtype)
-            return dx, None, None, None, None, None, None, None, None, None
+            return (dx,) + (None,) * 10
         dy2d = dy2d.contiguous()
         if dy2d.dtype != torch.bfloat16:
             dy2d = dy2d.to(torch.bfloat16)
         if ctx.needs_input_grad[0]:
-            wt = ext().transpose2d(wb)
+            wt = wt[0] if ctx.packed else ext().transpose2d(wb)
             if d_alias is not None and d_alias.dtype != torch.bfloat16:
                 d_alias = d_alias.to(torch.bfloat16)
             link = ctx.link
@@ -86,17 +94,17 @@
                 dw = dw.to(ctx.w_dtype)
         if ctx.needs_input_grad[2]:
             db = dy2d.float().sum(0)
-        return dx, dw, db, None, None, None, None, None, None, None
+        return (dx, dw, db) + (None,) * 8
 
 
 class _BNFromStatsFn(torch.autograd.Function):
 
     @staticmethod
     def forward(ctx, x, weight, bias, sums, running_mean, running_var,
-                momentum, eps, relu):
+                momentum, eps, relu, num_batches=None):
         y, mean, rstd, scale, shift = ext().batchnorm_fwd_from_sums(
             x, weight, bias, sums, running_mean, running_var, momentum, eps,
-            relu)
+            relu, num_batches)
         save_bn_for_backward(ctx, x, y, weight, mean, rstd, scale, shift,
                              relu)
         return y
@@ -104,7 +112,7 @@
     @staticmethod
     def backward(ctx, dy):
         dx, dw, db = bn_backward(ctx, dy)
-        return dx, dw, db, None, None, None, None, None, None
+        return dx, dw, db, None, None, None, None, None, None, None
 
 
 class _Stride2Fn(torch.autograd.Function):
@@ -140,6 +148,132 @@
     if cin % 64 != 0 or cout % 64 != 0:
         return False
     return x.dim() == 4 and x.is_contiguous(memory_format=torch.channels_last)
+
+
+def _weight_pack_disabled() -> bool:
+    return os.environ.get("DLA_NO_WEIGHT_PACK", "0") == "1"
+
+
+def _weight2d(w: torch.Tensor):
+    w2d = w.detach().reshape(w.shape[0], w.shape[1])
+    if w2d.is_contiguous() and w2d.data_ptr() == w.data_ptr():
+        return w2d
+    return None
+
+
+def _packable(m) -> bool:
+    return (isinstance(m, nn.Conv2d) and m.kernel_size == (1, 1) and
+            m.groups == 1 and m.padding == (0, 0) and
+            m.dilation == (1, 1) and m.stride in ((1, 1), (2, 2)) and
+            m.in_channels % 64 == 0 and m.out_channels % 64 == 0 and
+            _weight2d(m.weight) is not None)
+
+
+def torch_packer(pack):
+    out = []
+    for w in pack.weights:
+        wb = _weight2d(w).to(torch.bfloat16, copy=True)
+        out.append((wb, wb.t().contiguous()))
+    return out
+
+
+class WeightPack:
+
+    def __init__(self, root: nn.Module, packer=None):
+        self._root = weakref.ref(root)
+        self._packer = packer if packer is not None else WeightPack._pack_hip
+        self.refreshes = 0
+        self._collect()
+
+    def __deepcopy__(self, memo):
+        return None
+
+    def __reduce__(self):
+        return (type(None), ())
+
+    @classmethod
+    def attach(cls, root: nn.Module, packer=None):
+        pack = root.__dict__.get("_dla_weight_pack")
+        if pack is None:
+            pack = root._dla_weight_pack = cls(root, packer)
+        return pack
+
+    def _collect(self) -> None:
+        root = self._root()
+        self.convs = [m for m in root.modules() if _packable(m)] \
+            if root is not None else []
+        self.weights = [m.weight for m in self.convs]
+        for i, m in enumerate(self.convs):
+            m._dla_pack, m._dla_pack_index = self, i
+        self._sig = self._table = None
+        self.invalidate()
+
+    def invalidate(self) -> None:
+        self.keys = [None] * len(self.convs)
+        self.views = [None] * len(self.convs)
+
+    def __len__(self) -> int:
+        return len(self.convs)
+
+    def get(self, conv: nn.Conv2d):
+        if _weight_pack_disabled():
+            return None
+        i = conv.__dict__.get("_dla_pack_index", -1)
+        if not (0 <= i < len(self.convs) and self.convs[i] is conv and
+                self.weights[i] is conv.weight):
+            conv._dla_pack = None
+            self._collect()
+            if conv.__dict__.get("_dla_pack") is not self:
+                return None
+            i = conv._dla_pack_index
+        w = self.weights[i]
+        if self.keys[i] != (w.data_ptr(), w._version):
+            self.refresh()
+        return self.views[i]
+
+    def refresh(self) -> None:
+        self.views = list(self._packer(self))
+        self.keys = [(w.data_ptr(), w._version) for w in self.weights]
+        self.refreshes += 1
+
+    def _pack_hip(self):
+        ws = self.weights
+        sig = tuple((w.data_ptr(), w.dtype, w.device, tuple(w.stride()))
+                    for w in ws)
+        if sig != self._sig:
+            dev = next((w.device for w in ws if w.is_cuda), None)
+            srcs = [_weight2d(w) if w.device == dev and
+                    w.dtype in (torch.float32, torch.bfloat16) else None
+                    for w in ws]
+            self._slots, off = [], 0
+            for s in srcs:
+                n = s.numel() if s is not None else 0
+                self._slots.append((off, off + n) if n else None)
+                off += 2 * n
+            live = [k for k in self._slots if k is not None]
+            self._table = ext().weight_pack_table(
+                [s for s in srcs if s is not None], [k[0] for k in live],
+                [k[1] for k in live]) + (dev,) if live else None
+            self._sig = sig
+        if self._table is None:
+            return [None] * len(ws)
+        table, tiles, need, dev = self._table
+        arena = torch.empty(need, dtype=torch.bfloat16, device=dev)
+        ext().weight_pack_bf16(table, tiles, need, arena)
+        views = []
+        for w, k in zip(ws, self._slots):
+            if k is None:
+                views.append(None)
+                continue
+            N, K = w.shape[0], w.shape[1]
+            views.append((arena[k[0]:k[0] + N * K].view(N, K),
+                          arena[k[1]:k[1] + N * K].view(K, N)))
+        return views
+
+
+def packed_weight(conv: nn.Conv2d):
+    pack = conv.__dict__.get("_dla_pack")
+    return pack.get(conv) if pack is not None else None
 
 
 def _prep(x: torch.Tensor, conv: nn.Conv2d):
@@ -150,12 +284,13 @@
     x2d = _flatten_nhwc(x)
     w2d = conv.weight.reshape(conv.weight.shape[0], conv.weight.shape[1])
     bias = conv.bias.float() if conv.bias is not None else None
-    return x2d, w2d, bias, (B, H, W)
+    return x2d, w2d, bias, (B, H, W), packed_weight(conv)
 
 
 def conv1x1(x: torch.Tensor, conv: nn.Conv2d) -> torch.Tensor:
-    x2d, wb, bias, (B, H, W) = _prep(x, conv)
-    y2d = _Conv1x1Fn.apply(x2d, wb, bias, None, None, None, False, False)
+    x2d, wb, bias, (B, H, W), packed = _prep(x, conv)
+    y2d = _Conv1x1Fn.apply(x2d, wb, bias, None, None, None, False, False,
+                           False, None, packed)
     return _unflatten_nhwc(y2d, B, H, W)
 
 
@@ -173,33 +308,32 @@
             x.dtype != torch.bfloat16 or
             (link.mode != RELU_X and not pass_input)):
         link = None
-    x2d, wb, bias, (B, H, W) = _prep(x, conv)
+    x2d, wb, bias, (B, H, W), packed = _prep(x, conv)
     _fp32_running_stats(bn)
-    if bn.num_batches_tracked is not None:
-        bn.num_batches_tracked.add_(1)
-    momentum = bn._eaf() if hasattr(bn, "_eaf") else (bn.momentum or 0.0)
+    momentum, counter = bn_count_batch(bn)
     outs = _Conv1x1Fn.apply(x2d, wb, bias, None, None, None, False, True,
-                            pass_input, link)
+                            pass_input, link, packed)
     alias = _unflatten_nhwc(outs[2], B, H, W) if pass_input else None
-    return _unflatten_nhwc(outs[0], B, H, W), outs[1], momentum, alias
+    return (_unflatten_nhwc(outs[0], B, H, W), outs[1], momentum, alias,
+            counter)
 
 
 def conv1x1_bn(x: torch.Tensor, conv: nn.Conv2d, bn,
                pass_input: bool = False):
     relu = bool(getattr(bn, "relu", False))
     if bn.training:
-        y_raw, partials, momentum, alias = _conv1x1_train_stats(
+        y_raw, partials, momentum, alias, counter = _conv1x1_train_stats(
             x, conv, bn, pass_input)
         y = _BNFromStatsFn.apply(y_raw, bn.weight, bn.bias, partials,
                                  bn.running_mean, bn.running_var, momentum,
-                                 bn.eps, relu)
+                                 bn.eps, relu, counter)
         if relu:
             attach_relu_link(y)
         return (y, alias) if pass_input else y
     if pass_input:
         raise ValueError("conv1x1_bn: pass_input needs train mode")
 
-    x2d, wb, bias, (B, H, W) = _prep(x, conv)
+    x2d, wb, bias, (B, H, W), packed = _prep(x, conv)
     _fp32_running_stats(bn)
 
     if not bn.training:
@@ -209,12 +343,14 @@
         if not (torch.is_grad_enabled() and
                 (x.requires_grad or conv.weight.requires_grad or
                  bn.weight.requires_grad)):
+            wb = packed[0] if packed is not None else \
+                wb.to(torch.bfloat16).contiguous()
             y2d, _ = ext().conv1x1_fwd(
-                x2d.to(torch.bfloat16), wb.to(torch.bfloat16).contiguous(),
-                bias, scale.contiguous(), shift.contiguous(), None, relu,
-                False)
+                x2d.to(torch.bfloat16), wb, bias, scale.contiguous(),
+                shift.contiguous(), None, relu, False)
             return _unflatten_nhwc(y2d, B, H, W)
-        y2d = _Conv1x1Fn.apply(x2d, wb, bias, None, None, None, False, False)
+        y2d = _Conv1x1Fn.apply(x2d, wb, bias, None, None, None, False, False,
+                               False, None, packed)
         y = _unflatten_nhwc(y2d, B, H, W)
         y = y * scale.reshape(1, -1, 1, 1).to(y.dtype) + \
             shift.reshape(1, -1, 1, 1).to(y.dtype)
@@ -225,10 +361,10 @@
 
     @staticmethod
     def forward(ctx, x_raw, weight, bias, partials, running_mean,
-                running_var, momentum, eps, identity):
+                running_var, momentum, eps, identity, num_batches=None):
         out, mean, rstd = ext().bn_add_relu_fwd_from_sums(
             x_raw, weight, bias, partials, running_mean, running_var,
-            momentum, eps, identity)
+            momentum, eps, identity, num_batches)
         ctx.save_for_backward(x_raw, out, weight, mean, rstd)
         return out
 
@@ -244,7 +380,7 @@
         else:
             g, dx, dw, db = ext().bn_add_relu_bwd(dy, out, x_raw, weight,
                                                   mean, rstd)
-        return dx, dw, db, None, None, None, None, None, g
+        return dx, dw, db, None, None, None, None, None, g, None
 
 
 class _BNJoinDualFn(torch.autograd.Function):
@@ -252,12 +388,14 @@
     @staticmethod
     def forward(ctx, x_raw, weight, bias, partials, running_mean,
                 running_var, momentum, eps, xd_raw, weight_d, bias_d,
-                partials_d, running_mean_d, running_var_d, momentum_d, eps_d):
+                partials_d, running_mean_d, running_var_d, momentum_d, eps_d,
+                num_batches=None, num_batches_d=None):
         out, mean, rstd, mean_d, rstd_d = \
             ext().bn_add_relu_dual_fwd_from_sums(
                 x_raw, weight, bias, partials, running_mean, running_var,
                 momentum, eps, xd_raw, weight_d, bias_d, partials_d,
-                running_mean_d, running_var_d, momentum_d, eps_d)
+                running_mean_d, running_var_d, momentum_d, eps_d,
+                num_batches, num_batches_d)
         ctx.save_for_backward(x_raw, xd_raw, out, weight, mean, rstd,
                               weight_d, mean_d, rstd_d)
         return out
@@ -278,7 +416,7 @@
                 dy, out, x_raw, weight, mean, rstd, xd_raw, weight_d,
                 mean_d, rstd_d)
         return (dx, dw, db, None, None, None, None, None,
-                dxd, dwd, dbd, None, None, None, None, None)
+                dxd, dwd, dbd, None, None, None, None, None, None, None)
 
 
 def _fused_join_disabled() -> bool:
@@ -345,15 +483,16 @@
 def conv_bn_add_relu(x: torch.Tensor, conv: nn.Conv2d, bn, identity=None,
                      x_down=None, downsample=None) -> torch.Tensor:
     if can_fuse_join(x, conv, bn, identity, x_down, downsample):
-        y_raw, partials, momentum, _ = _conv1x1_train_stats(x, conv, bn)
+        y_raw, partials, momentum, _, counter = _conv1x1_train_stats(
+            x, conv, bn)
         if downsample is None:
             if identity.shape != y_raw.shape:
                 raise ValueError("conv_bn_add_relu: identity shape mismatch")
             return _attach_join_link(_BNJoinFn.apply(
                 y_raw, bn.weight, bn.bias, partials, bn.running_mean,
-                bn.running_var, momentum, bn.eps, identity))
+                bn.running_var, momentum, bn.eps, identity, counter))
         conv_d, bn_d = downsample[0], downsample[1]
-        yd_raw, partials_d, momentum_d, _ = _conv1x1_train_stats(
+        yd_raw, partials_d, momentum_d, _, counter_d = _conv1x1_train_stats(
             x_down, conv_d, bn_d)
         if yd_raw.shape != y_raw.shape:
             raise ValueError("conv_bn_add_relu: downsample shape mismatch")
@@ -361,7 +500,7 @@
             y_raw, bn.weight, bn.bias, partials, bn.running_mean,
             bn.running_var, momentum, bn.eps, yd_raw, bn_d.weight, bn_d.bias,
             partials_d, bn_d.running_mean, bn_d.running_var, momentum_d,
-            bn_d.eps))
+            bn_d.eps, counter, counter_d))
     from .activations import add_relu
 
     out = conv_bn(x, conv, bn)
@@ -476,10 +615,8 @@
         y = y * scale.reshape(1, -1, 1, 1).to(y.dtype) + \
             shift.reshape(1, -1, 1, 1).to(y.dtype)
         return torch.relu(y) if relu else y
-    if bn.num_batches_tracked is not None:
-        bn.num_batches_tracked.add_(1)
-    momentum = bn._eaf() if hasattr(bn, "_eaf") else (bn.momentum or 0.0)
+    momentum, counter = bn_count_batch(bn)
     y_raw, partials = _Conv3x3Fn.apply(x, conv.weight, True)
     return _BNFromStatsFn.apply(y_raw, bn.weight, bn.bias, partials,
                                 bn.running_mean, bn.running_var, momentum,
-                                bn.eps, relu)
+                                bn.eps, relu, counter)
diff --git a/deeplearning_amd/ops/stem.py b/deeplearning_amd/ops/stem.py
--- a/deeplearning_amd/ops/stem.py
+++ b/deeplearning_amd/ops/stem.py
@@ -6,14 +6,16 @@
 from torch import nn
 
 from ._ext import ext, use_hip
+from .batchnorm import bn_count_batch
 
 
 class _BNReluMaxPoolFn(torch.autograd.Function):
     @staticmethod
     def forward(ctx, x, weight, bias, running_mean, running_var, momentum,
-                eps):
+                eps, num_batches=None):
         pooled, slots, mean, rstd, scale, shift = ext().bn_relu_maxpool_fwd(
-            x, weight, bias, running_mean, running_var, momentum, eps)
+            x, weight, bias, running_mean, running_var, momentum, eps,
+            num_batches)
         ctx.save_for_backward(x, slots, weight, mean, rstd, scale, shift)
         return pooled
 
@@ -22,7 +24,7 @@
         x, slots, weight, mean, rstd, scale, shift = ctx.saved_tensors
         dx, dw, db = ext().bn_relu_maxpool_bwd(dpool, x, slots, weight, mean,
                                                rstd, scale, shift)
-        return dx, dw, db, None, None, None, None
+        return dx, dw, db, None, None, None, None, None
 
 
 def _fused_stem_disabled() -> bool:
@@ -63,7 +65,6 @@
     if bn.running_mean.dtype != torch.float32:
         bn.running_mean.data = bn.running_mean.data.float()
         bn.running_var.data = bn.running_var.data.float()
-    if bn.num_batches_tracked is not None:
-        bn.num_batches_tracked.add_(1)
+    momentum, counter = bn_count_batch(bn)
     return _BNReluMaxPoolFn.apply(x, bn.weight, bn.bias, bn.running_mean,
-                                  bn.running_var, bn._eaf(), bn.eps)
+                                  bn.running_var, momentum, bn.eps, counter)
```

Measured after the change: 10090 images/s, median of 6. About the same (+0.2%).
